# yabebalFantaye/MCEvidence

Measured on AMD Instinct MI355X. Metric: knn_queries_per_sec, higher is better.
Workload: dtype f16 filter + f64 refine (exact f64 results)

## Files before the change

### mcevidence_amd/csrc/capi_apo.hpp

```cpp
#pragma once
#include "sym_exchange.hpp"

namespace {

int pairs_once_plan(int64_t nr, int32_t d, int32_t kmax, Plan& p, bool quiet)
{
    if (kmax <= 1) return quiet ? MCE_ERR_INVALID : fail(MCE_ERR_INVALID, "kmax=%d must exceed k0=1", kmax);
    SameSetHint hint(true);
    const int rc = make_plan(nr, nr, d, kmax - 1, MCE_SELF_EXCLUDE, p);
    if (rc != MCE_OK) return rc;
    if (p.prune || !p.sym || p.twopass || !p.vh || !p.vh->launch_panel)
        return quiet ? MCE_ERR_INVALID : fail(MCE_ERR_INVALID, "pairs-once partition: this shape does not take the one-pass symmetric sweep");
    return MCE_OK;
}

struct PairsOnceShape {
    int nsplit = 1, panel = 0;
    size_t off_d = 0, off_i = 0;
    size_t total = 0;
};
PairsOnceShape pairs_once_shape(const Plan& p, int64_t nr, int32_t kmax, int32_t nparts)
{
    PairsOnceShape sh;
    const int nown = (p.nqblk + nparts - 1) / std::max(nparts, 1);
    const int env_split = env_pairs_once_split();
    const int env_panel = env_pairs_once_panel();
    int S = std::min(8, std::max(1, (1536 + nown - 1) / std::max(nown, 1)));
    if (env_split) S = env_split;
    const int def_panel = kSymPanelChunks[p.KST];
    int panel = S > 1 ? (int)std::max<int64_t>(8, std::min<int64_t>(def_panel, p.nchunk / (2 * S))) : 0;
    if (env_panel) panel = env_panel;
    sh.nsplit = S;
    sh.panel = panel;
    size_t off = p.total + dotp_ws_bytes(nr, kmax);
    if (S > 1) {
        off = align_up(off, 256);
        sh.off_d = off;
        off = align_up(off + (size_t)S * p.KCAP * (size_t)p.nq_pad * sizeof(double), 256);
        sh.off_i = off;
        off = align_up(off + (size_t)S * p.KCAP * (size_t)p.nq_pad * sizeof(int), 256);
    } else {
        sh.off_d = p.off_pd;
        sh.off_i = p.off_pi;
    }
    sh.total = off;
    return sh;
}
struct ApoCall { int64_t nr; int d, kmax, part, nparts, nsplit, panel, phase; };
std::mutex g_apo_mutex;
std::unordered_map<const void*, ApoCall> g_apo_calls;
int apo_step(const void* ws, int64_t nr, int d, int kmax, int part, int nparts, const PairsOnceShape& sh, int phase_from, int phase_to, int phase_set,
             const char* what)
{
    std::lock_guard<std::mutex> lk(g_apo_mutex);
    auto it = g_apo_calls.find(ws);
    if (phase_from > 0) {
        if (it == g_apo_calls.end())
            return fail(MCE_ERR_INVALID, "pairs-once partition: %s on a workspace that mce_pairs_once_prepare_dev has not prepared", what);
        const ApoCall& c = it->second;
        if (c.nr != nr || c.d != d || c.kmax != kmax || c.part != part || c.nparts != nparts || c.nsplit != sh.nsplit || c.panel != sh.panel)
            return fail(MCE_ERR_INVALID, "pairs-once partition: %s with other arguments than the workspace was prepared with (prepared: nr=%lld d=%d kmax=%d part %d "
                        "of %d, %d chains, panel %d)", what, (long long)c.nr, c.d, c.kmax, c.part, c.nparts, c.nsplit, c.panel);
        if (c.phase < phase_from || c.phase > phase_to)
            return fail(MCE_ERR_INVALID, "pairs-once partition: %s out of order (the calls are prepare, sweep, export, finish; this workspace stands after step %d)",
                        what, c.phase);
    }
    if (phase_set < 0) { if (it != g_apo_calls.end()) g_apo_calls.erase(it); }
    else g_apo_calls[ws] = ApoCall{nr, d, kmax, part, nparts, sh.nsplit, sh.panel, phase_set};
    return MCE_OK;
}
enum PairsOnceStep { kApoPrepare, kApoSweep, kApoExport, kApoFinish };
int pairs_once_begin(PairsOnceStep step, const void* ws, size_t ws_bytes, int64_t nr, int32_t d, int32_t kmax, int32_t part, int32_t nparts, Plan& p,
                     PairsOnceShape& sh)
{
    static const struct { int from, to, set; const char* what; } kSteps[4] = {{0, 0, 1, "prepare"}, {1, 1, 2, "sweep"}, {2, 3, 3, "export"},
                                                                               {2, 3, -1, "finish"}};
    int rc = pairs_once_plan(nr, d, kmax, p, false);
    if (rc != MCE_OK) return rc;
    if (nparts > p.nqblk || (step == kApoExport && nparts < 2))
        return step == kApoExport ? fail(MCE_ERR_INVALID, "part %d of %d", part, nparts)
                                  : fail(MCE_ERR_INVALID, "pairs-once partition: %d ranks for %d blocks", nparts, p.nqblk);
    sh = pairs_once_shape(p, nr, kmax, nparts);
    if (ws_bytes < sh.total)
        return step >= kApoExport ? fail(MCE_ERR_WORKSPACE, "workspace too small") : fail(MCE_ERR_WORKSPACE, "workspace too small: %zu < %zu", ws_bytes, sh.total);
    rc = apo_step(ws, nr, d, kmax, part, nparts, sh, kSteps[step].from, kSteps[step].to, kSteps[step].set, kSteps[step].what);
    if (rc != MCE_OK) return rc;
    p.apo = true; p.apo_nsplit = sh.nsplit; p.apo_panel = sh.panel; p.off_pd = sh.off_d; p.off_pi = sh.off_i;
    p.part = part; p.nparts = nparts;
    return MCE_OK;
}

__global__ __launch_bounds__(256) void pairs_once_fill_kernel(unsigned long long* __restrict__ p, int64_t n, unsigned long long v)
{
    for (int64_t i = (int64_t)blockIdx.x * 256 + threadIdx.x; i < n; i += (int64_t)gridDim.x * 256) p[i] = v;
}
__global__ __launch_bounds__(256) void pairs_once_row_gates_kernel(unsigned long long* __restrict__ thr, unsigned* __restrict__ rrow, float* __restrict__ rtile,
                                                                   const double* __restrict__ qinfo, const double* __restrict__ params, int64_t nq, int KST)
{
    const int64_t q = (int64_t)blockIdx.x * 256 + threadIdx.x;
    float R = 0.0f;
    if (q < nq) {
        R = mce::f16_row_gate_of(__longlong_as_double((long long)thr[q]), qinfo[2 * q], params, KST);
        rrow[q] = __float_as_uint(R);
    } else {
        thr[q] = 0x7FF0000000000000ull;
        rrow[q] = 0u;
    }
    float m = R;
#pragma unroll
    for (int o = 16; o >= 1; o >>= 1) m = fmaxf(m, __shfl_xor(m, o, 64));
    if ((threadIdx.x & 31) == 0) rtile[q >> 5] = m;
}

__global__ void pairs_once_poison_kernel(const int* __restrict__ err, double* __restrict__ dotp, int kmax)
{
    if (*err != 0 && (int)threadIdx.x < kmax) dotp[threadIdx.x] = __builtin_nan("");
}
__global__ __launch_bounds__(256) void pairs_once_check_kernel(const mce::SymEntry* __restrict__ recv, int64_t n, int qpb, int nqblk, int part, int nparts,
                                                               int* __restrict__ err)
{
    const int64_t i = (int64_t)blockIdx.x * 256 + threadIdx.x;
    if (i >= n) return;
    const int jb = recv[i].row / qpb;
    if (recv[i].row < 0 || jb >= nqblk || jb % nparts != part) *err = 1;
}

}

extern "C" {

int32_t mce_pairs_once_blocks(int64_t nr, int32_t d, int32_t kmax)
{
    Plan p;
    if (pairs_once_plan(nr, d, kmax, p, true) != MCE_OK) return 0;
    return p.nqblk;
}

size_t mce_pairs_once_workspace_bytes(int64_t nr, int32_t d, int32_t kmax, int32_t nparts)
{
    Plan p;
    if (nparts < 2 || pairs_once_plan(nr, d, kmax, p, true) != MCE_OK) return 0;
    return pairs_once_shape(p, nr, kmax, nparts).total;
}

int mce_pairs_once_prepare_dev(const double* dY, int64_t nr, int32_t d, int32_t kmax, int32_t part, int32_t nparts, size_t* bounds_offset,
                               int64_t* bounds_count, void* ws, size_t ws_bytes, void* stream)
{
    if (!dY || !ws || !bounds_offset || !bounds_count) return fail(MCE_ERR_INVALID, "null pointer argument");
    if (nparts < 2 || part < 0 || part >= nparts) return fail(MCE_ERR_INVALID, "part %d of %d (the pairs-once partition needs two ranks or more)", part, nparts);
    Plan p;
    PairsOnceShape sh;
    int rc = pairs_once_begin(kApoPrepare, ws, ws_bytes, nr, d, kmax, part, nparts, p, sh);
    if (rc != MCE_OK) return rc;
    hipStream_t st = static_cast<hipStream_t>(stream);
    char* wsc = static_cast<char*>(ws);
    p.apo_phase = 1;
    const unsigned long long inf_bits = 0x7FF0000000000000ull;
    hipLaunchKernelGGL(pairs_once_fill_kernel, dim3(1024), dim3(256), 0, st, reinterpret_cast<unsigned long long*>(wsc + p.off_sym + p.sl.thr), p.nq_pad, inf_bits);
    MCE_HIP(hipGetLastError());
    hipLaunchKernelGGL(pairs_once_fill_kernel, dim3(2048), dim3(256), 0, st, reinterpret_cast<unsigned long long*>(wsc + p.off_sym + p.sl.slots),
                       p.nq_pad * (int64_t)p.KCAP, inf_bits);
    MCE_HIP(hipGetLastError());
    if (sh.nsplit > 1) {
        static_assert(mce::f16_qpb(4) == 512, "one workgroup per block of list columns");
        hipLaunchKernelGGL(mce::sym_chain_init_kernel, dim3((unsigned)mce::apo_rank_count(p.nqblk, part, nparts)), dim3(512), 0, st,
                           reinterpret_cast<double*>(wsc + sh.off_d), reinterpret_cast<int*>(wsc + sh.off_i), p.nq_pad, p.KCAP, sh.nsplit, (int)part, (int)nparts);
        MCE_HIP(hipGetLastError());
    }
    SameSetHint hint(true);
    rc = run_search(p, dY, nr, dY, nr, d, kmax - 1, MCE_SELF_EXCLUDE, 0, wsc, st);
    if (rc != MCE_OK) return rc;
    *bounds_offset = p.off_sym + p.sl.thr;
    *bounds_count = p.nq_pad;
    return MCE_OK;
}

int mce_pairs_once_sweep_dev(const double* dY, int64_t nr, int32_t d, int32_t kmax, int32_t part, int32_t nparts, int64_t* d_counts,
                             int32_t* d_flags, void* ws, size_t ws_bytes, void* stream)
{
    if (!dY || !d_counts || !d_flags || !ws) return fail(MCE_ERR_INVALID, "null pointer argument");
    if (nparts < 2 || part < 0 || part >= nparts) return fail(MCE_ERR_INVALID, "part %d of %d (the pairs-once partition needs two ranks or more)", part, nparts);
    Plan p;
    PairsOnceShape sh;
    int rc = pairs_once_begin(kApoSweep, ws, ws_bytes, nr, d, kmax, part, nparts, p, sh);
    if (rc != MCE_OK) return rc;
    hipStream_t st = static_cast<hipStream_t>(stream);
    char* wsc = static_cast<char*>(ws);
    p.apo_phase = 2;
    const mce::KnnF16Args a = sym_args(p, wsc, nr, d, kmax - 1, 1);
    hipLaunchKernelGGL(pairs_once_row_gates_kernel, dim3((unsigned)(p.nq_pad / 256)), dim3(256), 0, st, a.sym.thr, a.sym.rrow, a.sym.rtile, a.qinfo, a.params, nr, p.KST);
    MCE_HIP(hipGetLastError());
    SameSetHint hint(true);
    rc = run_search(p, dY, nr, dY, nr, d, kmax - 1, MCE_SELF_EXCLUDE, 0, wsc, st);
    if (rc != MCE_OK) return rc;
    if (!p.sym_active) return fail(MCE_ERR_INVALID, "pairs-once partition: the sweep did not run");
    int* offs = reinterpret_cast<int*>(wsc + p.off_sym + p.sl.keys_a);
    static_assert(sizeof(long long) == sizeof(int64_t), "counts");
    hipLaunchKernelGGL(mce::apo_offsets_kernel, dim3(1), dim3(mce::kApoScanThreads), 0, st, a.sym.bucket_cnt, a.sym.bucket_flag, a.sym.cap, p.nqblk, (int)part,
                       (int)nparts, offs, reinterpret_cast<long long*>(d_counts), d_flags);
    MCE_HIP(hipGetLastError());
    return MCE_OK;
}

int mce_pairs_once_export_dev(int64_t nr, int32_t d, int32_t kmax, int32_t part, int32_t nparts, void* d_send, void* ws, size_t ws_bytes, void* stream)
{
    if (!ws) return fail(MCE_ERR_INVALID, "null pointer argument");
    Plan p;
    PairsOnceShape sh;
    const int rc = pairs_once_begin(kApoExport, ws, ws_bytes, nr, d, kmax, part, nparts, p, sh);
    if (rc != MCE_OK) return rc;
    if (!d_send) return MCE_OK;
    hipStream_t st = static_cast<hipStream_t>(stream);
    char* wsc = static_cast<char*>(ws);
    const mce::KnnF16Args a = sym_args(p, wsc, nr, d, kmax - 1, 1);
    const int* offs = reinterpret_cast<const int*>(wsc + p.off_sym + p.sl.keys_a);
    hipLaunchKernelGGL(mce::apo_export_kernel, dim3((unsigned)p.nqblk), dim3(256), 0, st, a.sym.bucket, offs, a.sym.cap, p.nqblk, (int)nparts,
                       static_cast<mce::SymEntry*>(d_send));
    MCE_HIP(hipGetLastError());
    return MCE_OK;
}

int mce_pairs_once_finish_dev(const double* dY, int64_t nr, int32_t d, int32_t kmax, int32_t part, int32_t nparts, const double* d_w,
                              const double* d_fs, const void* d_recv, int64_t nrecv, const int32_t* d_flags, double* d_dotp, void* ws,
                              size_t ws_bytes, void* stream)
{
    if (!dY || !d_w || !d_fs || !d_dotp || !d_flags || !ws || (nrecv > 0 && !d_recv)) return fail(MCE_ERR_INVALID, "null pointer argument");
    if (nparts < 2 || part < 0 || part >= nparts || nrecv < 0) return fail(MCE_ERR_INVALID, "part %d of %d, %lld entries", part, nparts, (long long)nrecv);
    Plan p;
    PairsOnceShape sh;
    int rc = pairs_once_begin(kApoFinish, ws, ws_bytes, nr, d, kmax, part, nparts, p, sh);
    if (rc != MCE_OK) return rc;
    hipStream_t st = static_cast<hipStream_t>(stream);
    char* wsc = static_cast<char*>(ws);
    const int K = kmax - 1;
    mce::KnnF16Args a = sym_args(p, wsc, nr, d, K, 1);
    const int nown = mce::apo_rank_count(p.nqblk, part, nparts);
    int* err = reinterpret_cast<int*>(wsc + p.off_sym + p.sl.keys_a) + p.nqblk + 1;
    MCE_HIP(mce::zero_async(err, sizeof(int), st));
    const int qpb = mce::f16_qpb(p.KCAP);
    if (nrecv > 0) {
        const unsigned nb = (unsigned)((nrecv + 255) / 256);
        hipLaunchKernelGGL(pairs_once_check_kernel, dim3(nb), dim3(256), 0, st, static_cast<const mce::SymEntry*>(d_recv), nrecv, qpb, p.nqblk, (int)part, (int)nparts, err);
        MCE_HIP(hipGetLastError());
        hipLaunchKernelGGL(mce::apo_import_kernel, dim3(nb), dim3(256), 0, st, static_cast<const mce::SymEntry*>(d_recv), nrecv, a.sym.bucket, a.sym.bucket_cnt,
                           a.sym.bucket_flag, a.sym.cap, qpb, p.nqblk, (int)part, (int)nparts);
        MCE_HIP(hipGetLastError());
    }
    hipLaunchKernelGGL(mce::apo_flags_kernel, dim3((unsigned)((nown + 255) / 256)), dim3(256), 0, st, d_flags, a.sym.bucket_flag, p.nqblk, (int)part, (int)nparts);
    MCE_HIP(hipGetLastError());
    a.seed_cfg = 0;
    MCE_HIP(p.vh->launch_sym_repair(a, st));
    if (sh.nsplit > 1 && nown > 0) {
        hipLaunchKernelGGL(mce::sym_chain_clear_kernel, dim3((unsigned)nown), dim3(512), 0, st, a.sym.bucket_flag, a.part_d, a.part_i, p.nq_pad, p.KCAP, sh.nsplit, (int)part, (int)nparts);
        MCE_HIP(hipGetLastError());
    }
    MCE_HIP(launch_sym_merge(p.KCAP, a.part_d, a.part_i, p.nq_pad, a.sym, part, p.nqblk, st, nparts));
    hipLaunchKernelGGL(mce::apo_iota_kernel, dim3((unsigned)((p.nqblk + 255) / 256)), dim3(256), 0, st, a.sym.done, p.nqblk);
    MCE_HIP(hipGetLastError());
    p.sym_qb_lo = 0; p.sym_qb_hi = p.nqblk; p.sym_active = true; p.L = sh.nsplit;
    double* partial = reinterpret_cast<double*>(wsc + p.total);
    rc = launch_merge(p, false, true, dY, dY, nr, d, K, MCE_SELF_EXCLUDE, 0, nullptr, nullptr, 1, (int)kmax, d_w, d_fs, partial, wsc, st);
    if (rc != MCE_OK) return rc;
    rc = finish_dotp(partial, (int64_t)nown * qpb, 1, kmax, d_dotp, st);
    if (rc != MCE_OK) return rc;
    hipLaunchKernelGGL(pairs_once_poison_kernel, dim3(1), dim3(64), 0, st, err, d_dotp, (int)kmax);
    MCE_HIP(hipGetLastError());
    return MCE_OK;
}

}
```

### mcevidence_amd/csrc/capi_common.hpp

```cpp
#pragma once
namespace {

thread_local char g_err[512] = "";
thread_local char g_last_kernel[256] = "";
thread_local int g_prof_on = 0;
thread_local std::vector<std::pair<hipEvent_t, hipEvent_t>> g_ev_pool;
thread_local size_t g_ev_used = 0;
thread_local size_t g_ev_calls = 0;
thread_local bool g_in_tail = false;
thread_local int g_split_depth = 0;
thread_local double g_last_prune_geom[3] = {0, 0, 0};
thread_local double g_last_flops_main = 0.0, g_last_flops_all = 0.0;
thread_local std::vector<std::pair<hipEvent_t, hipEvent_t>> g_evs_pool;
thread_local size_t g_evs_used = 0;

int fail(int code, const char* fmt, ...)
{
    va_list ap;
    va_start(ap, fmt);
    vsnprintf(g_err, sizeof(g_err), fmt, ap);
    va_end(ap);
    return code;
}

#define MCE_HIP(call)                                                                              \
    do {                                                                                           \
        hipError_t e_ = (call);                                                                    \
        if (e_ != hipSuccess)                                                                      \
            return fail(MCE_ERR_HIP, "%s failed: %s (%s:%d)", #call, hipGetErrorString(e_), __FILE__, __LINE__); \
    } while (0)

std::atomic<int> g_mode{0};
std::atomic<int> g_prune_mode{0};
struct Tuning {
    bool sym_kernel_f16 = false, tail_split = true, prune_prof = false, wide = true;
    int spin_limit = 1 << 21, sym_bucket = 0, sym_panel = 0, sym_seed_rows = 0, sym_seed_share = 2, sym_seed_mode = -1;
    int f16_seed_rows = -1, f16_seed_share = -1, f16_seed_tg = -1, rsplit = 0, panel_debug = 0, sym_chains = 0;
    size_t feed_wave_bytes = 0;
};
Tuning read_tuning()
{
    Tuning t;
    auto num = [](const char* name, int dflt) { const char* e = getenv(name); return e ? atoi(e) : dflt; };
    const char* e = getenv("MCE_SYM_KERNEL");
    t.sym_kernel_f16 = e && strcmp(e, "f16") == 0;
    t.spin_limit = num("MCE_SYM_SPIN_LIMIT", 1 << 21);
    t.sym_bucket = num("MCE_SYM_BUCKET", 0);
    t.sym_panel = num("MCE_SYM_PANEL", 0);
    t.sym_chains = num("MCE_SYM_CHAINS", 0);
    t.sym_seed_rows = num("MCE_SYM_SEED_ROWS", 0);
    t.sym_seed_share = num("MCE_SYM_SEED_SHARE", 2);
    t.sym_seed_mode = num("MCE_SYM_SEED_MODE", -1);
    t.f16_seed_rows = num("MCE_F16_SEED_ROWS", -1);
    t.f16_seed_share = num("MCE_F16_SEED_SHARE", -1);
    t.f16_seed_tg = num("MCE_F16_SEED_TG", -1);
    t.rsplit = num("MCE_RSPLIT", 0);
    t.tail_split = num("MCE_TAIL_SPLIT", 1) != 0;
    t.wide = num("MCE_WIDE", 1) != 0;
    t.panel_debug = num("MCE_PANEL_DEBUG", 0);
    t.prune_prof = getenv("MCE_PRUNE_PROF") != nullptr;
    if ((e = getenv("MCE_FEED_WAVE_BYTES"))) t.feed_wave_bytes = (size_t)std::strtoull(e, nullptr, 10);
    return t;
}
std::atomic<int> g_sym_mode{-1};
int sym_mode()
{
    int m = g_sym_mode.load();
    if (m < 0) {
        const char* e = getenv("MCE_SYM");
        m = e ? atoi(e) : 0;
        if (m < 0 || m > 2) m = 0;
        g_sym_mode.store(m);
    }
    return m;
}
const char* env_prune_heavy() { return getenv("MCE_PRUNE_HEAVY"); }
const char* env_prune_lists() { return getenv("MCE_PRUNE_LISTS"); }
const char* env_prune_times() { return getenv("MCE_PRUNE_TIMES"); }
bool env_long_on() { static const bool v = [] { const char* e = getenv("MCE_LONG"); return !(e && e[0] == '0'); }(); return v; }
bool env_deep_on() { static const bool v = [] { const char* e = getenv("MCE_DEEP"); return !(e && e[0] == '0'); }(); return v; }
int env_feed_eig() { static const int v = [] { const char* e = getenv("MCE_FEED_EIG"); return e && !strcmp(e, "hip") ? 2 : 1; }(); return v; }
bool env_feed_upload_async() { static const bool v = [] { const char* e = getenv("MCE_FEED_UPLOAD"); return e && !strcmp(e, "async"); }(); return v; }
int env_pairs_once_split() { static const int v = [] { const char* e = getenv("MCE_PAIRS_ONCE_SPLIT"); const int n = e ? atoi(e) : 0; return (n >= 1 && n <= 8) ? n : 0; }(); return v; }
int env_pairs_once_panel() { static const int v = [] { const char* e = getenv("MCE_PAIRS_ONCE_PANEL"); const int n = e ? atoi(e) : 0; return n >= 1 ? n : 0; }(); return v; }
struct CallOptions { int search = -1, prune = -1, sym = -1, same_set = -1, verify = -1, eig = 0; };
thread_local CallOptions t_opt;
thread_local std::vector<CallOptions> t_opt_stack;
int eff_search_mode() { return t_opt.search >= 0 ? t_opt.search : g_mode.load(); }
int eff_prune_mode() { return t_opt.prune >= 0 ? t_opt.prune : g_prune_mode.load(); }
int eff_sym_mode() { return t_opt.sym >= 0 ? t_opt.sym : sym_mode(); }
constexpr int kVerifyDefaultRows = 256;
constexpr int64_t kVerifyAlwaysFrom = 65536;
constexpr int kVerifySmallEvery = 8;
int default_verify_rows()
{
    static const int v = [] {
        const char* e = getenv("MCE_VERIFY");
        if (!e || !*e) return kVerifyDefaultRows;
        const long n = strtol(e, nullptr, 10);
        return (int)std::max<long>(0, std::min<long>(n, 1 << 20));
    }();
    return v;
}
bool verify_env_set() { static const bool s = [] { const char* e = getenv("MCE_VERIFY"); return e && *e; }(); return s; }
std::atomic<int> g_last_verify_rows{0};
thread_local unsigned t_small_search_count = 0;
int eff_verify(bool filter_path, int64_t nq)
{
    if (t_opt.verify >= 0) return t_opt.verify;
    if (!filter_path) return 0;
    if (nq < kVerifyAlwaysFrom && !verify_env_set() && (t_small_search_count++ % kVerifySmallEvery) != 0) return 0;
    return default_verify_rows();
}
constexpr int kSymAutoMinBlocks[5] = {0, 768, 257, 193, 193};
constexpr int kSymMaxChains = 8;
constexpr int kSymSeedMode[5] = {0, 0, 1, 1, 1};
constexpr int kSymPartitionMaxParts = 4;
thread_local int g_same_set_hint = -1;
thread_local size_t t_plan_cap = 0;
struct PlanCap {
    size_t prev;
    explicit PlanCap(size_t cap) : prev(t_plan_cap) { t_plan_cap = cap; }
    ~PlanCap() { t_plan_cap = prev; }
};
thread_local bool t_no_heavy = false;
struct NoHeavy {
    bool prev;
    NoHeavy() : prev(t_no_heavy) { t_no_heavy = true; }
    ~NoHeavy() { t_no_heavy = prev; }
};
struct SameSetHint {
    int prev;
    explicit SameSetHint(bool same) : prev(g_same_set_hint) { g_same_set_hint = same ? 1 : 0; }
    ~SameSetHint() { g_same_set_hint = prev; }
};
constexpr int kSymPanelChunks[5] = {0, 96, 256, 256, 256};
int sym_bucket_per_row(int K)
{
    const int b = read_tuning().sym_bucket;
    return b > 0 ? b : 6 * K + 24;
}
constexpr int64_t kPruneAutoMinQueries = 32768;
constexpr int64_t kPruneAutoMinRows[16] = {0, 100000, 100000, 100000, 100000, 125000, 150000, 250000, 500000, 0, 0, 0, 0, 0, 0, 0};

constexpr size_t kPoolMaxBytes = (size_t)64 << 20;
constexpr int kPoolSlots = 16;
struct PoolSlot { void* p = nullptr; size_t cap = 0; int dev = -1; bool busy = false; };
struct Pool {
    PoolSlot slot[kPoolSlots];
    PoolSlot& operator[](int i) { return slot[i]; }
    void release_idle()
    {
        for (int i = 0; i < kPoolSlots; ++i)
            if (slot[i].p && !slot[i].busy) {
                int cur = 0;
                (void)hipGetDevice(&cur);
                if (slot[i].dev != cur) (void)hipSetDevice(slot[i].dev);
                (void)hipFree(slot[i].p);
                if (slot[i].dev != cur) (void)hipSetDevice(cur);
                slot[i] = PoolSlot();
            }
    }
    ~Pool() { release_idle(); }
};
thread_local Pool g_pool;

struct PinnedArena {
    void* p = nullptr;
    size_t cap = 0;
    void release()
    {
        if (p) (void)hipHostFree(p);
        p = nullptr;
        cap = 0;
    }
    hipError_t reserve(size_t n)
    {
        if (n <= cap) return hipSuccess;
        release();
        const size_t c = std::max<size_t>(n + n / 2, (size_t)64 << 10);
        hipError_t e = hipHostMalloc(&p, c, hipHostMallocPortable);
        if (e != hipSuccess) { p = nullptr; return e; }
        cap = c;
        return hipSuccess;
    }
    ~PinnedArena() { release(); }
};
thread_local PinnedArena g_pinned;

thread_local const double* g_last_params = nullptr;

struct DevBuf {
    void* p = nullptr;
    int slot = -1;
    ~DevBuf()
    {
        if (p && g_last_params >= static_cast<const double*>(p) &&
            reinterpret_cast<const char*>(g_last_params) < static_cast<const char*>(p) + bytes)
            g_last_params = nullptr;
        if (slot >= 0) g_pool[slot].busy = false;
        else if (p) (void)hipFree(p);
    }
    size_t bytes = 0;
    hipError_t alloc(size_t n)
    {
        if (n == 0) n = 1;
        bytes = n;
        if (n <= kPoolMaxBytes) {
            int dev = 0;
            (void)hipGetDevice(&dev);
            int pick = -1;
            for (int i = 0; i < kPoolSlots; ++i)
                if (!g_pool[i].busy && g_pool[i].p && g_pool[i].dev == dev && g_pool[i].cap >= n &&
                    (pick < 0 || g_pool[i].cap < g_pool[pick].cap)) pick = i;
            if (pick < 0)
                for (int i = 0; i < kPoolSlots; ++i)
                    if (!g_pool[i].busy) {
                        if (g_pool[i].p) { (void)hipFree(g_pool[i].p); g_pool[i].p = nullptr; g_pool[i].cap = 0; }
                        const size_t cap = n + n / 4;
                        hipError_t e = hipMalloc(&g_pool[i].p, cap);
                        if (e != hipSuccess) { g_pool[i].p = nullptr; return e; }
                        g_pool[i].cap = cap;
                        g_pool[i].dev = dev;
                        pick = i;
                        break;
                    }
            if (pick >= 0) {
                g_pool[pick].busy = true;
                slot = pick;
                p = g_pool[pick].p;
                return hipSuccess;
            }
        }
        return hipMalloc(&p, n);
    }
    template <class T> T* as() { return static_cast<T*>(p); }
};

}
```

### mcevidence_amd/csrc/capi_plan.hpp

```cpp
#pragma once
namespace {

using mce::kMaxDevices;
constexpr int kAssumedCUs = 256;

size_t align_up(size_t x, size_t a) { return (x + a - 1) / a * a; }

constexpr bool kPruneHeavyDefault = false;
constexpr int kPruneHeavyMinBlocks = 64, kPruneHeavyCount = 700, kPruneHeavyMaxShare = 16, kPruneHeavyMinCount = 32, kPruneHeavyMaxRounds = 60;
constexpr double kPruneHeavyFullRounds = 10.0;
constexpr int kPruneHeavySplit = 4, kPruneHeavyMaxSplit = 8;
constexpr int kPruneWaveQueries = mce::kHQT * 32;
constexpr int kWideMinBlocks = 480;
bool prune_heavy_enabled()
{
    if (t_no_heavy) return false;
    const char* e = env_prune_heavy();
    return kPruneHeavyDefault || (e && *e && strcmp(e, "0") != 0);
}
static_assert(mce::kPruneWavesPerBlock == mce::kHWaves, "prune.hip orders kHWaves waves per query block");

constexpr int kRefineMargin = 2;
struct Plan {
    const mce::KnnVariant* v = nullptr;
    const mce::KnnF16Variant* vh = nullptr;
    const mce::KnnDeepVariant* vd = nullptr;
    bool filter() const { return vh != nullptr || vd != nullptr; }
    const mce::KnnLongVariant* vl = nullptr;
    size_t off_xf = 0, off_xn = 0;
    bool generic = false;
    int KST = 0;
    size_t off_yh = 0, off_xh = 0, off_qinfo = 0, off_params = 0;
    int KS = 0, KCAP = 0, QT = 0, CT = 0;
    int64_t nchunk = 0;
    int64_t nrow_pad = 0;
    int nqblk = 0;
    int64_t nq_pad = 0;
    int rsplit = 1;
    int L = 4;
    size_t off_yf = 0, off_pd = 0, off_pi = 0, off_center = 0, off_msum = 0, total = 0;
    double cost = 0.0;
    int ksel = 0;
    bool twopass = false;
    bool wide_ok = false;
    bool prune = false;
    bool kd_ready = false;
    int part = 0, nparts = 1;
    int sym_qb_lo = 0, sym_qb_hi = 0;
    bool apo = false;
    int apo_phase = 0;
    int apo_nsplit = 1;
    int apo_panel = 0;
    int64_t pl_nr = 0;
    mce::PruneLayout pl;
    size_t off_prune = 0;
    size_t off_heavy = 0;
    int heavy_max = 0;
    bool sym = false;
    bool sym_active = false;
    mce::SymLayout sl;
    size_t off_sym = 0;
    int sym_nsplit = 1;
    int sym_panel = 0;
};

const mce::KnnVariant* variant_for(int KS, int kcap_idx)
{
    switch (kcap_idx) {
        case 0: return &mce::g_knn_kcap4[mce::mfma_variant_index(KS)];
        case 1: return &mce::g_knn_kcap8[mce::mfma_variant_index(KS)];
        case 2: return &mce::g_knn_kcap12[mce::mfma_variant_index(KS)];
        case 3: return &mce::g_knn_kcap16[mce::mfma_variant_index(KS)];
        case 4: return &mce::g_knn_kcap24[mce::mfma_variant_index(KS)];
        default: return &mce::g_knn_kcap32[mce::mfma_variant_index(KS)];
    }
}

int sweep_seed_cfg(int64_t cps, int CT, int kneed)
{
    const Tuning t = read_tuning();
    if (t.f16_seed_rows >= 0 || t.f16_seed_share >= 0 || t.f16_seed_tg >= 0)
        return mce::f16_seed_cfg(cps, CT, kneed, t.f16_seed_rows >= 0 ? t.f16_seed_rows : MCE_H_SEED_ROWS, t.f16_seed_share >= 0 ? t.f16_seed_share : MCE_H_SEED_SHARE,
                                 t.f16_seed_tg >= 0 ? t.f16_seed_tg : MCE_H_SEED_TG);
    for (int share = MCE_H_SEED_SHARE; share >= 2; share /= 2)
        for (int tg = MCE_H_SEED_TG; tg >= 2; tg /= 2)
            if (const int cfg = mce::f16_seed_cfg(cps, CT, kneed, MCE_H_SEED_ROWS, share, tg)) return cfg;
    return 0;
}

template <class V> const V* by_kcap(int ki, const V* t4, const V* t8, const V* t12, const V* t16) { return ki == 0 ? t4 : ki == 1 ? t8 : ki == 2 ? t12 : t16; }

double split_cost(const Plan& p, bool filt, int64_t nr, int32_t K, int r)
{
    const double n_r = (double)nr / r;
    const double lnf = 1.0 + std::log(std::max(1.0, n_r / K));
    const double block = filt ? 64.0 * p.QT * p.KST * (n_r / 32.0) + 300.0 * 32.0 * p.QT * K * lnf
                              : 256.0 * p.KS * (n_r / 16.0) + 1000.0 * 32.0 * K * lnf;
    const double rounds = std::ceil((double)p.nqblk * r / kAssumedCUs);
    return rounds * block;
}

int make_plan(int64_t nq, int64_t nr, int32_t d, int32_t K, int32_t self_mode, Plan& p)
{
    if (nq < 0 || nr < 1 || d < 1 || K < 1) return fail(MCE_ERR_INVALID, "invalid sizes nq=%lld nr=%lld d=%d K=%d", (long long)nq, (long long)nr, d, K);
    if (self_mode < 0 || self_mode > 2) return fail(MCE_ERR_INVALID, "invalid self_mode %d", self_mode);
    if (d > mce::kGenMaxDim) return fail(MCE_ERR_DIM_RANGE, "d=%d exceeds the supported maximum %d", d, mce::kGenMaxDim);
    if (K > mce::kGenMaxK) return fail(MCE_ERR_K_RANGE, "K=%d exceeds the supported maximum %d", K, mce::kGenMaxK);
    const int64_t usable = (self_mode == MCE_SELF_EXCLUDE) ? nr - 1 : nr;
    if (K > usable)
        return fail(MCE_ERR_K_RANGE, "Expected n_neighbors <= n_samples_fit, but n_neighbors = %d, n_samples_fit = %lld", K, (long long)usable);
    if (nr >= (int64_t)1 << 31) return fail(MCE_ERR_INVALID, "nr=%lld exceeds 2^31-1 reference rows", (long long)nr);

    const bool wide_f64 = d > MCE_MAX_DIM && d <= mce::kWideMaxDim && K <= MCE_MAX_K;
    if (env_long_on() && d >= mce::kLongMinDim && d <= mce::kLongMaxDim && K <= MCE_MAX_K) {
        p.ksel = std::min<int>(K + kRefineMargin, MCE_MAX_K);
        p.vl = &mce::g_knn_long[p.ksel <= 8 ? 0 : (p.ksel <= 16 ? 1 : 2)];
        p.v = nullptr;
        p.vh = nullptr;
        p.KCAP = p.vl->kcap;
        p.CT = p.vl->ct;
        p.QT = mce::kLongQT;
        p.KS = mce::long_ksp(d);
        p.nqblk = (int)std::max<int64_t>(1, (nq + mce::kLongQPB - 1) / mce::kLongQPB);
        p.nq_pad = (int64_t)p.nqblk * mce::kLongQPB;
        const int64_t rows_per_chunk = (int64_t)p.CT * 16;
        p.nchunk = (nr + rows_per_chunk - 1) / rows_per_chunk;
        p.nrow_pad = p.nchunk * rows_per_chunk;
        int best_r = 1;
        double best_c = 1e300;
        const int rmax = (int)std::min<int64_t>(mce::kMaxLists, p.nchunk);
        for (int r = 1; r <= rmax; ++r) {
            const double c = std::ceil((double)p.nqblk * r / kAssumedCUs) * (std::ceil((double)p.nchunk / r) + 16.0);
            if (c < best_c * 0.98) { best_c = c; best_r = r; }
        }
        p.rsplit = best_r;
        p.L = p.rsplit;
        p.cost = best_c;
        p.pl_nr = nr;
        size_t off = 0;
        p.off_pd = off;
        off = align_up(off + (size_t)p.L * p.KCAP * (size_t)p.nq_pad * sizeof(double), 256);
        p.off_pi = off;
        off = align_up(off + (size_t)p.L * p.KCAP * (size_t)p.nq_pad * sizeof(int), 256);
        p.off_center = off;
        off = align_up(off + (size_t)(d + 4) * sizeof(double), 256);
        p.off_msum = off;
        off = align_up(off + (size_t)mce::kLongMeanBlocks * (size_t)d * sizeof(double), 256);
        p.off_yf = off;
        off = align_up(off + (size_t)p.nrow_pad * (size_t)p.KS * 4 * sizeof(double), 256);
        p.off_xf = off;
        off = align_up(off + (size_t)p.nq_pad * (size_t)p.KS * 4 * sizeof(double), 256);
        p.off_xn = off;
        off = align_up(off + (size_t)p.nq_pad * sizeof(double), 256);
        p.total = off + 256;
        return MCE_OK;
    }
    if ((d > MCE_MAX_DIM && !wide_f64) || K > MCE_MAX_K) {
        p.generic = true;
        p.v = nullptr;
        p.vh = nullptr;
        p.KCAP = K;
        p.rsplit = 1;
        p.L = 1;
        p.nqblk = (int)std::max<int64_t>(1, (nq + mce::kGenThreads - 1) / mce::kGenThreads);
        p.nq_pad = (int64_t)p.nqblk * mce::kGenThreads;
        size_t off = 0;
        p.off_pd = off;
        off = align_up(off + (size_t)K * (size_t)p.nq_pad * sizeof(double), 256);
        p.off_pi = off;
        off = align_up(off + (size_t)K * (size_t)p.nq_pad * sizeof(int), 256);
        p.off_center = off;
        off = align_up(off + (size_t)nq * K * sizeof(double), 256);
        p.off_msum = off;
        p.total = off + 256;
        return MCE_OK;
    }
    p.KS = mce::mfma_ks_for(d);
    int ki = 0;
    while (ki < mce::kNumKcap - 1 && mce::kKcapList[ki] < K) ++ki;
    p.KCAP = mce::kKcapList[ki];
    const bool f16 = !wide_f64 && (eff_search_mode() != 1) && mce::f16_supported(d, K);
    const bool deep = wide_f64 && (eff_search_mode() != 1) && mce::deep_supported(d, K) && env_deep_on();
    const bool filt = f16 || deep;
    p.vd = nullptr;
    int qpb, rows_per_tile;
    if (filt) {
        if (K > 16) {
            p.twopass = true;
            ki = 3;
            p.KCAP = 16;
        }
        if (deep) {
            p.KST = mce::deep_ksteps(d);
            p.vd = &by_kcap(ki, mce::g_knn_deep_kcap4, mce::g_knn_deep_kcap8, mce::g_knn_deep_kcap12, mce::g_knn_deep_kcap16)[p.KST == 5 ? 0 : (p.KST == 6 ? 1 : 2)];
            p.vh = nullptr;
            p.QT = mce::kHQT;
            p.CT = p.vd->ct;
        } else {
            p.KST = mce::f16_ksteps(d);
            p.vh = &by_kcap(ki, mce::g_knn_f16_kcap4, mce::g_knn_f16_kcap8, mce::g_knn_f16_kcap12, mce::g_knn_f16_kcap16)[p.KST - 1];
            p.QT = p.vh->qt;
            p.CT = p.vh->ct;
        }
        p.v = nullptr;
        qpb = mce::f16_qpb(p.KCAP);
        rows_per_tile = 32;
    } else {
        p.ksel = std::min<int>(K + kRefineMargin, MCE_MAX_K);
        p.pl_nr = nr;
        ki = 0;
        while (ki < mce::kNumKcap - 1 && mce::kKcapList[ki] < p.ksel) ++ki;
        p.KCAP = mce::kKcapList[ki];
        p.v = variant_for(p.KS, ki);
        p.vh = nullptr;
        p.QT = p.v->qt;
        p.CT = p.v->ct;
        qpb = mce::queries_per_block(p.QT);
        rows_per_tile = 16;
    }
    p.nqblk = (int)std::max<int64_t>(1, (nq + qpb - 1) / qpb);
    p.wide_ok = f16 && !p.twopass && p.KST == 1 && p.vh->launch_wide && p.nqblk >= kWideMinBlocks && nr <= ((int64_t)1 << 25) && read_tuning().wide;
    if (p.wide_ok && (p.nqblk & 1)) p.nqblk += 1;
    p.nq_pad = (int64_t)p.nqblk * qpb;
    const int64_t rows_per_chunk = (int64_t)p.CT * rows_per_tile;
    p.nchunk = (nr + rows_per_chunk - 1) / rows_per_chunk;
    p.nrow_pad = p.nchunk * rows_per_chunk;

    if (f16 && !p.twopass && p.KST == 1 && d <= mce::kPruneMaxDim && p.vh->launch_prune && nq > 0 &&
        p.nrow_pad <= ((int64_t)1 << mce::kHRelBits) && (int64_t)p.nqblk * p.nchunk <= mce::kPruneMaxPairs) {
        const int pm = eff_prune_mode();
        p.prune = pm == 2 || (pm == 0 && kPruneAutoMinRows[d] > 0 && nr >= kPruneAutoMinRows[d] && nq >= kPruneAutoMinQueries &&
                                           nq >= nr / 8);
    }
    if (p.prune) {
        p.CT = mce::kHPruneChunkTiles;
        p.nchunk = (nr + p.CT * 32 - 1) / (p.CT * 32);
        p.nrow_pad = p.nchunk * p.CT * 32;
        if (p.nrow_pad > ((int64_t)1 << mce::kHRelBits)) p.prune = false;
        if (!p.prune) {
            p.CT = p.vh->ct;
            p.nchunk = (nr + rows_per_chunk - 1) / rows_per_chunk;
            p.nrow_pad = p.nchunk * rows_per_chunk;
        }
    }
    int best_r = 1;
    double best_c = 1e300;
    const int rmax = (int)std::min<int64_t>(p.twopass ? mce::kMaxLists / 2 : mce::kMaxLists, p.nchunk);
    const int rmin = f16 ? (int)((nr + ((int64_t)1 << mce::kHRelBits) - 1) >> mce::kHRelBits) : 1;
    if (deep && p.nrow_pad > ((int64_t)1 << mce::kHRelBits))
        return fail(MCE_ERR_INVALID, "reference set too large for the fp16-filter path at d = %d (nr=%lld): use search mode 1", d, (long long)nr);
    if (rmin > rmax) return fail(MCE_ERR_INVALID, "reference set too large for the fp16-filter path (nr=%lld)", (long long)nr);
    for (int r = std::max(1, rmin); r <= rmax; ++r) {
        const double c = split_cost(p, filt, nr, K, r);
        if (c < best_c * 0.98) { best_c = c; best_r = r; }
    }
    if (f16 && !p.twopass && p.nqblk <= kAssumedCUs) {
        const int kneed = K + 1;
        for (int r = std::min(rmax, kAssumedCUs / p.nqblk); r >= std::max(1, rmin); --r)
            if (sweep_seed_cfg(p.nchunk / r, p.CT, kneed)) { best_r = r; break; }
    }
    if (deep && p.nqblk <= kAssumedCUs) {
        for (int r = std::min(rmax, kAssumedCUs / p.nqblk); r >= 1; --r)
            if ((p.nchunk / r) * p.CT >= 4 * (K + 1)) { best_r = r; break; }
    }
    if (const int r = read_tuning().rsplit) {
        if (r >= std::max(1, rmin) && r <= rmax) best_r = r;
    }
    if (p.prune) best_r = 1;
    p.rsplit = best_r;
    p.cost = split_cost(p, filt, nr, K, best_r);
    auto layout = [&]() {
    p.L = p.twopass ? 2 * p.rsplit : p.rsplit;

    size_t off = 0;
    p.off_yf = off;
    if (filt) {
        p.off_yh = off;
        off = align_up(off + (size_t)p.nrow_pad * (size_t)(16 * p.KST) * 2, 256);
        p.off_xh = off;
        off = align_up(off + (size_t)p.nq_pad * (size_t)(16 * p.KST) * 2, 256);
        p.off_qinfo = off;
        off = align_up(off + (size_t)p.nq_pad * 2 * sizeof(double), 256);
        p.off_params = off;
        off = align_up(off + (size_t)mce::HP_COUNT * sizeof(double), 256);
    } else {
        off = align_up(off + (size_t)p.nrow_pad * (size_t)(4 * p.KS) * sizeof(double), 256);
    }
    if (f16 && (!p.twopass || p.vh->launch_panel_lower) && !p.prune && nq == nr && p.vh->launch_sym && p.nqblk >= 2 && p.nrow_pad <= ((int64_t)1 << mce::kHSymRowBits)) {
        const int sm = eff_sym_mode();
        p.sym = sm == 2 || (sm == 0 && p.nqblk >= kSymAutoMinBlocks[p.KST] * ((p.KST == 1 && p.KCAP == 16) ? 2 : 1));
        if (g_same_set_hint == 0 || (g_same_set_hint < 0 && t_opt.same_set == 0)) p.sym = false;
    }
    p.sym_nsplit = 1;
    p.sym_panel = 0;
    if (p.sym && !p.twopass) {
        const Tuning tun = read_tuning();
        int S = 1;
        if (tun.sym_chains >= 1) S = std::min(tun.sym_chains, kSymMaxChains);
        p.sym_nsplit = S;
        if (S > 1) p.sym_panel = (int)std::max<int64_t>(8, std::min<int64_t>(kSymPanelChunks[p.KST], p.nchunk / (2 * S)));
    }
    const int l_alloc = std::max(p.L, p.sym_nsplit);
    p.off_pd = off;
    off = align_up(off + (size_t)l_alloc * p.KCAP * (size_t)p.nq_pad * sizeof(double), 256);
    p.off_pi = off;
    off = align_up(off + (size_t)l_alloc * p.KCAP * (size_t)p.nq_pad * sizeof(int), 256);
    p.off_center = off;
    off = align_up(off + (size_t)3 * mce::kMaxDimPad * sizeof(double), 256);
    p.off_msum = off;
    off = align_up(off + (size_t)mce::kMeanBlocks * mce::kStatStride * sizeof(double), 256);
    if (p.prune) {
        mce::prune_layout(nq, p.nq_pad, p.nqblk, nr, p.nrow_pad, p.nchunk, d, p.pl);
        p.pl_nr = nr;
        p.off_prune = off;
        off = align_up(off + p.pl.total, 256);
        if (nq == nr && p.nqblk >= kPruneHeavyMinBlocks && prune_heavy_enabled()) {
            p.heavy_max = std::max(p.nqblk * mce::kHWaves / kPruneHeavyMaxShare, kPruneHeavyMinCount);
            p.off_heavy = off;
            off = align_up(off + (size_t)p.heavy_max * kPruneWaveQueries * (kPruneHeavyMaxSplit - 1) * p.KCAP * (sizeof(double) + sizeof(int)), 256);
        }
    }
    if (p.sym) {
        mce::sym_layout(nr, p.nq_pad, p.nqblk, d, p.KCAP, mce::f16_qpb(p.KCAP), sym_bucket_per_row(std::min<int>(K, p.KCAP)), p.sl);
        p.off_sym = off;
        off = align_up(off + p.sl.total, 256);
    }
    p.total = off;
    };
    layout();
    while (t_plan_cap && p.total > t_plan_cap && p.rsplit > std::max(1, rmin)) {
        p.rsplit -= 1;
        layout();
    }
    return MCE_OK;
}

size_t dotp_ws_bytes(int64_t nq, int32_t kmax)
{
    const int64_t nb = (nq + mce::kRedThreads - 1) / mce::kRedThreads;
    return align_up((size_t)std::max<int64_t>(nb, 1) * (size_t)kmax * sizeof(double), 256);
}

int plan_for_workspace(int64_t nq, int64_t nr, int32_t d, int32_t K, int32_t self_mode, size_t ws_bytes, size_t extra, bool same_set_fallback,
                       Plan& p, std::optional<NoHeavy>& nh)
{
    int rc = make_plan(nq, nr, d, K, self_mode, p);
    if (rc != MCE_OK) return rc;
    if (same_set_fallback && ws_bytes < p.total + extra && p.sym) {
        g_same_set_hint = 0;
        rc = make_plan(nq, nr, d, K, self_mode, p);
        if (rc != MCE_OK) return rc;
    }
    if (ws_bytes < p.total + extra && p.heavy_max > 0) {
        nh.emplace();
        rc = make_plan(nq, nr, d, K, self_mode, p);
        if (rc != MCE_OK) return rc;
    }
    if (ws_bytes < p.total + extra) return fail(MCE_ERR_WORKSPACE, "workspace too small: %zu < %zu", ws_bytes, p.total + extra);
    return MCE_OK;
}

}
```

### mcevidence_amd/csrc/capi_search.hpp

```cpp
#pragma once
namespace {

double ln_unit_ball(int d) { return 0.5 * d * std::log(M_PI) - std::lgamma(1.0 + 0.5 * d); }

hipError_t launch_sym_merge(int KCAP, double* pd, int* pi, int64_t nq_pad, const mce::SymParams& sym, int qb_lo, int qb_hi, hipStream_t st, int stride = 1)
{
    const int nb = qb_hi > qb_lo ? (qb_hi - qb_lo + stride - 1) / stride : 0;
    if (nb <= 0) return hipSuccess;
    const dim3 g((unsigned)nb), b(mce::kSymMergeThreads);
    static_assert(mce::kSymMergeThreads == mce::f16_qpb(4), "one merge block per query block");
    switch (KCAP) {
        case 4: hipLaunchKernelGGL(mce::sym_merge_kernel<4>, g, b, 0, st, pd, pi, nq_pad, sym.bucket_cnt, sym.bucket_flag, sym.bucket, sym.cap, qb_lo, stride); break;
        case 8: hipLaunchKernelGGL(mce::sym_merge_kernel<8>, g, b, 0, st, pd, pi, nq_pad, sym.bucket_cnt, sym.bucket_flag, sym.bucket, sym.cap, qb_lo, stride); break;
        case 12: hipLaunchKernelGGL(mce::sym_merge_kernel<12>, g, b, 0, st, pd, pi, nq_pad, sym.bucket_cnt, sym.bucket_flag, sym.bucket, sym.cap, qb_lo, stride); break;
        default: hipLaunchKernelGGL(mce::sym_merge_kernel<16>, g, b, 0, st, pd, pi, nq_pad, sym.bucket_cnt, sym.bucket_flag, sym.bucket, sym.cap, qb_lo, stride); break;
    }
    return hipGetLastError();
}

struct KernelBracket {
    bool on = false; hipStream_t st = nullptr;
    hipError_t begin() const
    {
        if (!on) return hipSuccess;
        if (g_ev_used == g_ev_pool.size()) {
            hipEvent_t e0, e1;
            if (const hipError_t e = hipEventCreate(&e0)) return e;
            if (const hipError_t e = hipEventCreate(&e1)) return e;
            g_ev_pool.emplace_back(e0, e1);
        }
        return hipEventRecord(g_ev_pool[g_ev_used].first, st);
    }
    hipError_t end() const
    {
        if (!on) return hipSuccess;
        if (const hipError_t e = hipEventRecord(g_ev_pool[g_ev_used].second, st)) return e;
        ++g_ev_used;
        if (!g_in_tail) ++g_ev_calls;
        return hipSuccess;
    }
};
struct SearchBracket {
    hipStream_t st; bool on;
    SearchBracket(hipStream_t s, bool o) : st(s), on(o)
    {
        if (!on) return;
        if (g_evs_used == g_evs_pool.size()) {
            hipEvent_t e0, e1;
            if (hipEventCreate(&e0) != hipSuccess || hipEventCreate(&e1) != hipSuccess) { on = false; return; }
            g_evs_pool.emplace_back(e0, e1);
        }
        (void)hipEventRecord(g_evs_pool[g_evs_used].first, st);
    }
    ~SearchBracket() { if (on) { (void)hipEventRecord(g_evs_pool[g_evs_used].second, st); ++g_evs_used; } }
};

size_t list_set(const Plan& p, int set) { return (size_t)set * p.KCAP * (size_t)p.nq_pad; }

mce::KnnF16Args f16_args(const Plan& p, char* ws, const double* X, int64_t nq, const double* Y, int64_t nr, int32_t d, int32_t K, int self_exclude,
                         int64_t self_offset)
{
    mce::KnnF16Args a;
    a.Yh = ws + p.off_yh; a.nchunk_total = p.nchunk; a.rsplit = p.rsplit; a.Xh = ws + p.off_xh;
    a.qinfo = reinterpret_cast<const double*>(ws + p.off_qinfo); a.params = reinterpret_cast<const double*>(ws + p.off_params);
    a.X = X; a.Y = Y; a.nq = nq; a.nr = nr; a.D = d; a.nq_pad = p.nq_pad; a.nqblk = p.nqblk;
    a.self_exclude = self_exclude; a.self_offset = self_offset; a.ksel = K;
    a.part_d = reinterpret_cast<double*>(ws + p.off_pd); a.part_i = reinterpret_cast<int*>(ws + p.off_pi);
    return a;
}
mce::KnnF16Args sym_args(const Plan& p, char* ws, int64_t n, int32_t d, int32_t K, int self_exclude)
{
    char* const sw = ws + p.off_sym;
    const double* rows = reinterpret_cast<const double*>(sw + p.sl.Ys);
    mce::KnnF16Args a = f16_args(p, ws, rows, n, rows, n, d, K, self_exclude, 0);
    a.rsplit = 1;
    a.rperm = reinterpret_cast<const int*>(sw + p.sl.perm);
    a.sym.thr = reinterpret_cast<unsigned long long*>(sw + p.sl.thr);
    a.sym.rrow = reinterpret_cast<unsigned*>(sw + p.sl.rrow);
    a.sym.rtile = reinterpret_cast<float*>(sw + p.sl.rtile);
    a.sym.slots = reinterpret_cast<unsigned long long*>(sw + p.sl.slots);
    a.sym.bucket_cnt = reinterpret_cast<int*>(sw + p.sl.bucket_cnt);
    a.sym.bucket_flag = reinterpret_cast<int*>(sw + p.sl.bucket_flag);
    a.sym.bucket = reinterpret_cast<mce::SymEntry*>(sw + p.sl.bucket);
    a.sym.cap = p.sl.cap;
    a.sym.done = reinterpret_cast<int*>(sw + p.sl.done);
    const Tuning tun = read_tuning();
    a.sym.panel = tun.sym_panel > 0 ? tun.sym_panel : kSymPanelChunks[p.KST];
    return a;
}

struct F16Search {
    const double* sX = nullptr;
    const double* sY = nullptr;
    mce::PruneOut po;
    bool use_sym = false;
};

struct Search {
    Plan& p;
    const double* dX; int64_t nq; const double* dY; int64_t nr; int32_t d, K;
    int32_t self_mode; int64_t self_offset; char* ws; hipStream_t st;
    int phase;
    double* pd; int* pi;
    double* center; double* msum;
    int self_exclude;
    KernelBracket kb;
    int generic(), long_rows(), deep(), fp64();
    int f16_prepare(F16Search& f), pruned(const F16Search& f), symmetric(), f16_sweep(const F16Search& f);
};

int Search::generic()
{
    const size_t lds = mce::generic_lds_bytes();
    hipLaunchKernelGGL(mce::knn_generic_kernel, dim3((unsigned)p.nqblk), dim3(mce::kGenThreads), 0, st, dX, nq, dY, nr, (int)d,
                       (int)K, p.nq_pad, self_exclude, self_offset, pd, pi);
    MCE_HIP(hipGetLastError());
    snprintf(g_last_kernel, sizeof(g_last_kernel), "knn_generic_kernel grid=%d block=%d lds=%zu", p.nqblk, mce::kGenThreads, lds);
    return MCE_OK;
}

int Search::long_rows()
{
    const int threads = 256;
    double* yf = reinterpret_cast<double*>(ws + p.off_yf);
    double* xf = reinterpret_cast<double*>(ws + p.off_xf);
    double* xn = reinterpret_cast<double*>(ws + p.off_xn);
    hipLaunchKernelGGL(mce::pack_refs_kernel, dim3((unsigned)((p.nrow_pad + threads - 1) / threads)), dim3(threads), 0, st, dY, nr, (int)d, p.KS, p.nrow_pad, center, yf);
    MCE_HIP(hipGetLastError());
    const int64_t qe = p.nq_pad * (int64_t)p.KS;
    hipLaunchKernelGGL(mce::long_pack_queries_kernel, dim3((unsigned)((qe + 255) / 256)), dim3(256), 0, st, dX, nq, (int)d, p.KS, p.nq_pad, center, xf);
    MCE_HIP(hipGetLastError());
    hipLaunchKernelGGL(mce::long_query_norms_kernel, dim3((unsigned)((p.nq_pad + 255) / 256)), dim3(256), 0, st, dX, nq, (int)d, p.nq_pad, center, xn);
    MCE_HIP(hipGetLastError());
    mce::LongArgs a;
    a.Yf = yf; a.Xf = xf; a.xn = xn;
    a.nchunk_total = p.nchunk; a.rsplit = p.rsplit; a.KSP = p.KS; a.KSB = mce::long_ksb(d);
    a.nq = nq; a.nq_pad = p.nq_pad; a.nqblk = p.nqblk;
    a.self_exclude = self_exclude; a.self_offset = self_offset; a.ksel = p.ksel > K ? p.ksel : K;
    a.part_d = pd; a.part_i = pi;
    MCE_HIP(kb.begin());
    MCE_HIP(p.vl->launch(a, st));
    MCE_HIP(kb.end());
    snprintf(g_last_kernel, sizeof(g_last_kernel), "%s grid=%d block=%d lds=%zu qt=%d ct=%d rsplit=%d ksp=%d", p.vl->name, p.nqblk * p.rsplit, mce::kThreads,
             p.vl->lds_bytes, p.QT, p.CT, p.rsplit, p.KS);
    g_last_flops_main = g_last_flops_all = (double)p.nq_pad * (double)p.nrow_pad * 2.0 * 4.0 * p.KS;
    return MCE_OK;
}

int Search::deep()
{
    _Float16* yh = reinterpret_cast<_Float16*>(ws + p.off_yh);
    _Float16* xh = reinterpret_cast<_Float16*>(ws + p.off_xh);
    double* qinfo = reinterpret_cast<double*>(ws + p.off_qinfo);
    double* params = reinterpret_cast<double*>(ws + p.off_params);
    MCE_HIP(mce::zero_async(params, mce::HP_COUNT * sizeof(double), st));
    const bool separate_queries = !(dX >= dY && dX + (size_t)nq * d <= dY + (size_t)nr * d);
    hipLaunchKernelGGL(mce::f16_radius_rows_kernel, dim3((unsigned)std::min<int64_t>((nr + 255) / 256, 2048)), dim3(256), 0, st, dY, nr, (int)d, center, params);
    MCE_HIP(hipGetLastError());
    if (separate_queries && nq > 0) {
        hipLaunchKernelGGL(mce::f16_radius_rows_kernel, dim3((unsigned)std::min<int64_t>((nq + 255) / 256, 2048)), dim3(256), 0, st, dX, nq, (int)d, center, params);
        MCE_HIP(hipGetLastError());
    }
    hipLaunchKernelGGL(mce::f16_scale_from_radius_kernel, dim3(1), dim3(1), 0, st, params);
    MCE_HIP(hipGetLastError());
    const int64_t rows_per_block = 4 * (64 / (2 * p.KST));
    const int64_t pack_blocks = std::min<int64_t>((p.nrow_pad + rows_per_block - 1) / rows_per_block, 2048);
    hipLaunchKernelGGL(mce::f16_pack_refs_kernel, dim3((unsigned)pack_blocks), dim3(256), 0, st, dY, nr, (int)d, p.KST, p.nrow_pad, center, params, yh);
    MCE_HIP(hipGetLastError());
    hipLaunchKernelGGL(mce::f16_pack_queries_kernel, dim3((unsigned)((p.nq_pad + rows_per_block - 1) / rows_per_block)), dim3(256), 0, st,
                       dX, nq, p.nq_pad, (int)d, p.KST, center, params, xh, qinfo);
    MCE_HIP(hipGetLastError());
    mce::DeepArgs a;
    a.Yh = yh; a.Xh = xh; a.qinfo = qinfo; a.params = params; a.X = dX; a.Y = dY; a.part_d = pd; a.part_i = pi;
    a.nq = nq; a.nr = nr; a.nq_pad = p.nq_pad; a.self_offset = self_offset; a.nchunk_total = p.nchunk;
    a.D = d; a.ksel = K; a.self_exclude = self_exclude; a.nqblk = p.nqblk; a.rsplit = p.rsplit;
    const Tuning tun = read_tuning();
    a.debug = tun.panel_debug;
    const int64_t tiles_split = (p.nchunk / p.rsplit) * p.CT;
    const int64_t want = (tun.f16_seed_rows >= 0 ? tun.f16_seed_rows : MCE_H_SEED_ROWS) / 32;
    auto tg_for = [&](int G) {
        int64_t tg = std::min<int64_t>(want, tiles_split / 4) / G;
        if (tg < 1) tg = std::min<int64_t>(want, tiles_split / 2) / G;
        return (int)std::max<int64_t>(tg, 0);
    };
    a.seed_tg = tg_for(K + a.self_exclude);
    MCE_HIP(kb.begin());
    double seed_rows = (double)a.seed_tg * (K + a.self_exclude) * 32.0 * p.rsplit;
    if (p.twopass) {
        const int tg2 = a.seed_tg;
        a.ksel = 16;
        a.seed_groups = 16 + a.self_exclude;
        a.seed_tg = tg_for(a.seed_groups);
        const int tg1 = a.seed_tg;
        MCE_HIP(p.vd->launch(a, st));
        a.lo_d = pd; a.lo_i = pi;
        a.part_d = pd + list_set(p, p.rsplit); a.part_i = pi + list_set(p, p.rsplit);
        a.ksel = K - 16;
        a.seed_groups = K + a.self_exclude;
        a.seed_tg = tg2;
        MCE_HIP(p.vd->launch_lower(a, st));
        seed_rows = ((double)tg1 * (16 + a.self_exclude) + (double)tg2 * (K + a.self_exclude)) * 32.0 * p.rsplit;
    } else {
        MCE_HIP(p.vd->launch(a, st));
    }
    MCE_HIP(kb.end());
    g_last_flops_main = g_last_flops_all = (double)p.nq_pad * ((p.twopass ? 2.0 : 1.0) * (double)p.nrow_pad + seed_rows) * 2.0 * 16.0 * p.KST;
    snprintf(g_last_kernel, sizeof(g_last_kernel), "%s grid=%d block=%d lds=%zu qt=%d ct=%d rsplit=%d%s seed=%dx%d", p.vd->name, p.nqblk * p.rsplit, mce::kHThreads,
             p.vd->lds_bytes, p.QT, p.CT, p.rsplit, p.twopass ? " two passes" : "", K + a.self_exclude, a.seed_tg);
    return MCE_OK;
}

int Search::f16_prepare(F16Search& f)
{
    _Float16* yh = reinterpret_cast<_Float16*>(ws + p.off_yh);
    _Float16* xh = reinterpret_cast<_Float16*>(ws + p.off_xh);
    double* qinfo = reinterpret_cast<double*>(ws + p.off_qinfo);
    double* params = reinterpret_cast<double*>(ws + p.off_params);
    double* box_y = center + mce::kMaxDimPad;
    double* box_x = center + 2 * mce::kMaxDimPad;
    if (phase != 2) MCE_HIP(mce::zero_async(params, mce::HP_COUNT * sizeof(double), st));
    bool separate_queries = !(dX >= dY && dX + (size_t)nq * d <= dY + (size_t)nr * d);
    f.sX = dX; f.sY = dY;
    f.use_sym = p.sym && dX == dY && nq == nr && self_offset == 0 && g_split_depth == 0;
    if (f.use_sym) {
        if (phase != 2) MCE_HIP(mce::sym_prepare(dY, nr, (int)d, center, p.nq_pad, ws + p.off_sym, p.sl, st));
        f.sX = f.sY = reinterpret_cast<const double*>(ws + p.off_sym + p.sl.Ys);
        separate_queries = false;
    }
    if (p.prune) {
        const bool same_set = (dX == dY && nq == nr);
        MCE_HIP(mce::prune_prepare(dX, nq, dY, nr, (int)d, same_set, mce::f16_qpb(p.KCAP), p.CT * 32, p.nq_pad, p.nqblk, p.nrow_pad,
                                   p.nchunk, ws + p.off_prune, p.pl, st, f.po, p.kd_ready && same_set));
        f.sX = f.po.Xs; f.sY = f.po.Ys;
        separate_queries = separate_queries && !same_set;
    }
    if (separate_queries) {
        hipLaunchKernelGGL(mce::col_stats_partial_kernel, dim3(mce::kMeanBlocks), dim3(mce::kMeanThreads), 0, st, dX, nq, (int)d, msum);
        MCE_HIP(hipGetLastError());
        hipLaunchKernelGGL(mce::f16_box_about_kernel, dim3(1), dim3(64), 0, st, msum, (int)d, center, box_x);
        MCE_HIP(hipGetLastError());
    }
    if (phase == 2) return MCE_OK;
    hipLaunchKernelGGL(mce::f16_scale_kernel, dim3(1), dim3(64), 0, st, box_y, separate_queries ? box_x : (const double*)nullptr, params);
    MCE_HIP(hipGetLastError());
    const int64_t rows_per_block = 4 * (64 / (2 * p.KST));
    const int64_t pack_blocks = std::min<int64_t>((p.nrow_pad + rows_per_block - 1) / rows_per_block, 2048);
    const bool one_pass = f.sX == f.sY && nq == nr && p.nq_pad <= p.nrow_pad;
    hipLaunchKernelGGL(mce::f16_pack_refs_kernel, dim3((unsigned)pack_blocks), dim3(256), 0, st,
                       f.sY, nr, (int)d, p.KST, p.nrow_pad, center, params, yh, one_pass ? xh : (_Float16*)nullptr, one_pass ? qinfo : (double*)nullptr,
                       one_pass ? p.nq_pad : (int64_t)0);
    MCE_HIP(hipGetLastError());
    if (!one_pass) {
        hipLaunchKernelGGL(mce::f16_pack_queries_kernel, dim3((unsigned)((p.nq_pad + rows_per_block - 1) / rows_per_block)), dim3(256), 0, st,
                           f.sX, nq, p.nq_pad, (int)d, p.KST, center, params, xh, qinfo);
        MCE_HIP(hipGetLastError());
    }
    return MCE_OK;
}

int Search::pruned(const F16Search& f)
{
    const mce::PruneOut& po = f.po;
    mce::KnnF16Args a = f16_args(p, ws, f.sX, nq, f.sY, nr, d, K, self_exclude, self_offset);
    a.clist = po.clist; a.cdist = po.cdist; a.list_len = (int)p.nchunk; a.rperm = po.rperm; a.qperm = po.qperm;
    a.tbox_r = po.tbox_r; a.tbox_q = po.tbox_q; a.cbox_r = po.cbox_r; a.border = po.border;
    const int nw_total = p.nqblk * mce::kHWaves;
    if (p.nparts > 1) { a.qblk0 = p.part; a.qblk_stride = p.nparts; a.nqblk_run = (nw_total - p.part + p.nparts - 1) / p.nparts; }
    const int nblk_run = a.nqblk_run ? a.nqblk_run : nw_total;
    int hv_n = 0, hv_S = 1;
    if (p.heavy_max > 0 && dX == dY && nq == nr) {
        const double rounds = (double)nblk_run / 2048.0;
        const char* hv_env = env_prune_heavy();
        if ((kPruneHeavyDefault || (hv_env && !strcmp(hv_env, "auto"))) && rounds < kPruneHeavyMaxRounds) {
            const double fr = std::min(1.0, kPruneHeavyFullRounds / std::max(rounds, 1.0));
            hv_n = std::min(std::max((int)(kPruneHeavyCount * fr), kPruneHeavyMinCount), std::min(p.heavy_max, nblk_run));
            hv_S = kPruneHeavySplit;
        }
        if (const char* e = hv_env) {
            int n_ = hv_n, s_ = kPruneHeavySplit;
            if (sscanf(e, "%d,%d", &n_, &s_) >= 1) { hv_n = std::min(std::max(n_, 0), std::min(p.heavy_max, nblk_run)); hv_S = std::min(std::max(s_, 1), kPruneHeavyMaxSplit); }
        }
        if (hv_n == 0 || hv_S == 1) { hv_n = 0; hv_S = 1; }
    }
    double* hv_d = reinterpret_cast<double*>(ws + p.off_heavy);
    int* hv_i = reinterpret_cast<int*>(hv_d + (size_t)p.heavy_max * kPruneWaveQueries * (kPruneHeavyMaxSplit - 1) * p.KCAP);
    a.seed_cfg = hv_n | (hv_S << 24);
    a.lo_d = hv_n ? hv_d : nullptr; a.lo_i = hv_n ? hv_i : nullptr;
    const char* times_file = env_prune_times();
    const size_t n_wg = (size_t)(nblk_run + hv_n * (hv_S - 1));
    DevBuf wg_times;
    if (times_file && *times_file) { MCE_HIP(wg_times.alloc(n_wg * sizeof(float))); a.wg_us = wg_times.as<float>(); }
    MCE_HIP(kb.begin());
    const char* force_lists = env_prune_lists();
    mce::knn_f16_launch_fn short_fn = nullptr;
    int short_lc = 0;
    if (p.vh->launch_prune_short && K <= p.vh->prune_short_lc) { short_fn = p.vh->launch_prune_short; short_lc = p.vh->prune_short_lc; }
    else if (p.vh->launch_prune_short2 && K <= p.vh->prune_short_lc2) { short_fn = p.vh->launch_prune_short2; short_lc = p.vh->prune_short_lc2; }
    const bool short_lists = short_fn && !(force_lists && !strcmp(force_lists, "long"));
    MCE_HIP(short_lists ? short_fn(a, st) : p.vh->launch_prune(a, st));
    MCE_HIP(kb.end());
    if (a.wg_us) {
        std::vector<float> us(n_wg);
        MCE_HIP(hipStreamSynchronize(st));
        MCE_HIP(hipMemcpy(us.data(), a.wg_us, n_wg * sizeof(float), hipMemcpyDeviceToHost));
        if (FILE* fh = fopen(times_file, "wb")) {
            const int hdr[4] = {(int)n_wg, hv_n, hv_S, 1};
            fwrite(hdr, sizeof(int), 4, fh);
            fwrite(us.data(), sizeof(float), n_wg, fh);
            fclose(fh);
        }
    }
    if (hv_n) {
        const unsigned fb = (unsigned)(((int64_t)hv_n * kPruneWaveQueries + mce::kRedThreads - 1) / mce::kRedThreads);
        hipLaunchKernelGGL(mce::prune_heavy_fold_kernel, dim3(fb), dim3(mce::kRedThreads), 0, st, pd, pi, p.nq_pad, p.KCAP, hv_d, hv_i, hv_n, hv_S,
                           kPruneWaveQueries, po.border, a.qblk0, a.qblk_stride);
        MCE_HIP(hipGetLastError());
    }
    g_last_params = a.params;
    g_last_flops_main = g_last_flops_all = -1.0;
    g_last_prune_geom[0] = p.nqblk; g_last_prune_geom[1] = (double)p.nchunk; g_last_prune_geom[2] = p.CT;
    snprintf(g_last_kernel, sizeof(g_last_kernel), "%s pruned grid=%d block=64 lds=%zu qt=%d ct=%d chunks=%lld heavy=%dx%d lists=%d", p.vh->name,
             nblk_run + hv_n * (hv_S - 1), mce::f16_prune_lds_bytes(p.KST, d, short_lists ? short_lc : p.KCAP), p.QT, p.CT, (long long)p.nchunk, hv_n,
             hv_S, short_lists ? short_lc : p.KCAP);
    return MCE_OK;
}

int sym_units_and_flops(const Plan& p, const mce::PanelGeom& g, bool panel_kernel, int64_t nr, int panel)
{
    int units = mce::sym_unit_count(p.nqblk, mce::kHWaves * mce::kHQT, panel * p.CT, (int)((nr + 31) / 32) + (int)(((nr + 31) / 32) & 1));
    double tiles = 0.0;
    if (panel_kernel) {
        units = mce::panel_unit_count(g);
        for (int u = 0; g_prof_on && u < units; ++u) {
            int pp, aa, lo, hi;
            mce::panel_unit_decode(u, g, pp, aa);
            mce::panel_unit_tiles(pp, aa, g, lo, hi);
            tiles += hi - lo;
        }
    } else {
        const double tpb = mce::kHWaves * mce::kHQT, T = (double)((nr + 31) / 32);
        for (int b = 0; b < p.nqblk; ++b) tiles += std::min(tpb * (b + 1), T);
    }
    g_last_flops_main = tiles * 16.0 * 1024.0 * 32.0 * p.KST;
    return units;
}

int Search::symmetric()
{
    char* const sw = ws + p.off_sym;
    mce::KnnF16Args a = sym_args(p, ws, nr, d, K, self_exclude);
    const Tuning tun = read_tuning();
    const int seed_rows = tun.sym_seed_rows > 0 ? tun.sym_seed_rows : (p.KST == 1 ? 65536 : 32768) * (p.apo && p.nparts >= 4 ? 2 : 1);
    const int seed_share = tun.sym_seed_share;
    auto sym_seed_for = [&](int kk) {
        int cfg = mce::f16_seed_cfg(p.nchunk, p.CT, kk + a.self_exclude, seed_rows, seed_share, MCE_H_SEED_TG);
        for (int tg = MCE_H_SEED_TG / 2; cfg == 0 && tg >= 1; tg /= 2)
            cfg = mce::f16_seed_cfg(p.nchunk, p.CT, kk + a.self_exclude, seed_rows, seed_share, tg);
        if (cfg) cfg |= ((tun.sym_seed_mode >= 0 ? tun.sym_seed_mode : kSymSeedMode[p.KST]) & 3) << 28;
        return cfg;
    };
    const int qb_lo = p.nparts > 1 && !p.apo ? (int)((int64_t)p.nqblk * p.part / p.nparts) : 0;
    const int qb_hi = p.nparts > 1 && !p.apo ? (int)((int64_t)p.nqblk * (p.part + 1) / p.nparts) : p.nqblk;
    p.sym_qb_lo = qb_lo; p.sym_qb_hi = qb_hi;
    const bool panel_kernel = !tun.sym_kernel_f16 || p.nparts > 1 || p.twopass;
    mce::PanelGeom geom;
    geom.qb_lo = qb_lo; geom.qb_hi = qb_hi; geom.tpb = mce::kHWaves * mce::kHQT; geom.ct = p.CT; geom.tpp = a.sym.panel * p.CT; geom.sym_on = 1;
    geom.ntiles = (int)((nr + 31) / 32) + (int)(((nr + 31) / 32) & 1);
    const bool apo = p.apo && p.nparts > 1 && !p.twopass && panel_kernel;
    const bool chains1 = !apo && p.nparts == 1 && panel_kernel && !p.twopass && p.sym_nsplit > 1;
    if (apo) { geom.blk_first = p.part; geom.blk_stride = p.nparts; }
    if (apo || chains1) {
        const int pn = apo ? p.apo_panel : p.sym_panel;
        if (pn > 0 && (apo || tun.sym_panel <= 0)) { a.sym.panel = pn; geom.tpp = a.sym.panel * p.CT; }
        geom.nsplit = std::max(1, apo ? p.apo_nsplit : p.sym_nsplit);
        if (geom.nsplit > 1) {
            a.sym.done = reinterpret_cast<int*>(sw + p.sl.keys_b);
            MCE_HIP(mce::zero_async(a.sym.done, (size_t)p.nqblk * geom.nsplit * sizeof(int), st));
            if (!apo) {
                hipLaunchKernelGGL(mce::sym_chain_init_kernel, dim3((unsigned)p.nqblk), dim3(512), 0, st, pd, pi, p.nq_pad, p.KCAP, geom.nsplit, 0, 1);
                MCE_HIP(hipGetLastError());
            }
        }
    }
    const bool unit_table = apo || geom.nsplit > 1;
    const int npass = p.twopass ? 2 : 1;
    int seed_used = 0;
    for (int pass = 0; pass < npass; ++pass) {
        const bool lower = pass == 1;
        const int Kp = !p.twopass ? K : (lower ? K - 16 : 16);
        double* const pdp = pd + (lower ? list_set(p, 1) : 0);
        int* const pip = pi + (lower ? list_set(p, 1) : 0);
        if (lower) {
            MCE_HIP(mce::zero_async(a.sym.bucket_cnt, (size_t)3 * p.nqblk * sizeof(int), st));
            a.sym.slot_stride = p.KCAP;
        }
        a.ksel = lower ? K : Kp;
        a.seed_cfg = sym_seed_for(a.ksel);
        a.part_d = pdp; a.part_i = pip;
        a.qblk0 = qb_lo;
        a.nqblk_run = qb_hi - qb_lo;
        if (apo) {
            a.qblk0 = p.part; a.qblk_stride = p.nparts; a.nqblk_run = mce::apo_rank_count(p.nqblk, p.part, p.nparts);
        }
        if (a.nqblk_run > 0 && phase != 2) MCE_HIP((lower ? p.vh->launch_sym_pre32 : p.vh->launch_sym_pre)(a, st));
        a.qblk0 = 0; a.qblk_stride = 1; a.nqblk_run = 0;
        if (phase == 1) return MCE_OK;
        if (pass == 0) seed_used = a.seed_cfg;
        a.seed_cfg = 0;
        a.ksel = Kp;
        a.lo_d = lower ? pd : nullptr; a.lo_i = lower ? pi : nullptr;
        if (pass == 0) MCE_HIP(kb.begin());
        if (panel_kernel) {
            mce::PanelArgs pa;
            pa.Yh = static_cast<const _Float16*>(a.Yh); pa.Xh = static_cast<const _Float16*>(a.Xh); pa.qinfo = a.qinfo; pa.params = a.params;
            pa.X = a.X; pa.Y = a.Y; pa.rperm = a.rperm;
            pa.part_d = pdp; pa.part_i = pip; pa.nq = nq; pa.nr = nr; pa.nq_pad = p.nq_pad; pa.self_offset = 0;
            pa.D = d; pa.ksel = Kp; pa.self_exclude = a.self_exclude; pa.spin_limit = tun.spin_limit;
            pa.sym = a.sym; pa.debug = tun.panel_debug; pa.geom = geom; pa.lo_d = a.lo_d; pa.lo_i = a.lo_i;
            if (unit_table) {
                const int nun = mce::panel_unit_count(geom);
                if ((size_t)nun * sizeof(mce::PanelUnit) > (size_t)p.nq_pad * sizeof(int)) return fail(MCE_ERR_INVALID, "symmetric sweep: %d units do not fit the table", nun);
                mce::PanelUnit* tab = reinterpret_cast<mce::PanelUnit*>(sw + p.sl.vals_a);
                if (nun > 0) {
                    hipLaunchKernelGGL(mce::panel_unit_table_kernel, dim3((unsigned)((nun + 255) / 256)), dim3(256), 0, st, geom, nun, tab);
                    MCE_HIP(hipGetLastError());
                }
                pa.units = tab;
            }
            MCE_HIP((lower ? p.vh->launch_panel_lower : p.vh->launch_panel)(pa, st));
        } else {
            MCE_HIP(p.vh->launch_sym(a, st));
        }
        if (pass == 0) MCE_HIP(kb.end());
        if (apo) break;
        MCE_HIP((lower ? p.vh->launch_sym_repair_lower : p.vh->launch_sym_repair)(a, st));
        if (geom.nsplit > 1) {
            hipLaunchKernelGGL(mce::sym_chain_clear_kernel, dim3((unsigned)p.nqblk), dim3(512), 0, st, a.sym.bucket_flag, pdp, pip, p.nq_pad, p.KCAP, geom.nsplit, 0, 1);
            MCE_HIP(hipGetLastError());
        }
        MCE_HIP(launch_sym_merge(p.KCAP, pdp, pip, p.nq_pad, a.sym, qb_lo, qb_hi, st));
    }
    p.sym_active = true;
    p.L = geom.nsplit > 1 ? geom.nsplit : npass;
    const int sym_units = sym_units_and_flops(p, geom, panel_kernel, nr, a.sym.panel);
    g_last_flops_all = g_last_flops_main + (double)(seed_used & 0xffff) * p.CT * (double)(qb_hi - qb_lo) * 16.0 * 1024.0 * 32.0 * p.KST;
    snprintf(g_last_kernel, sizeof(g_last_kernel), "%s symmetric%s%s%s grid=%d block=%d lds=%zu qt=%d ct=%d panel=%d seed=%dx%d/%d bucket=%d", p.vh->name, panel_kernel ? " panel-kernel" : "",
             p.twopass ? " two passes" : "", geom.blk_stride > 1 ? " pairs-once" : (geom.nsplit > 1 ? " chains" : ""), sym_units,
             mce::kHThreads, panel_kernel ? p.vh->lds_bytes_panel : p.vh->lds_bytes_sym, p.QT, p.CT, a.sym.panel, seed_used & 0xffff, (seed_used >> 16) & 0xfff, (seed_used >> 28) & 3, p.sl.cap);
    return MCE_OK;
}

int Search::f16_sweep(const F16Search& f)
{
    mce::KnnF16Args a = f16_args(p, ws, f.sX, nq, f.sY, nr, d, K, self_exclude, self_offset);
    auto seed_cfg = [&](int ksel) { return sweep_seed_cfg(p.nchunk / p.rsplit, p.CT, ksel + a.self_exclude); };
    MCE_HIP(kb.begin());
    if (p.twopass) {
        a.ksel = 16;
        a.seed_cfg = seed_cfg(16);
        MCE_HIP(p.vh->launch(a, st));
        a.lo_d = pd; a.lo_i = pi;
        a.part_d = pd + list_set(p, p.rsplit); a.part_i = pi + list_set(p, p.rsplit);
        a.ksel = K - 16;
        a.seed_cfg = 0;
        MCE_HIP(p.vh->launch_lower(a, st));
    } else {
        a.seed_cfg = seed_cfg(K);
        if (p.wide_ok) MCE_HIP(p.vh->launch_wide(a, st));
        else MCE_HIP(p.vh->launch(a, st));
    }
    MCE_HIP(kb.end());
    const int seed_first = p.twopass ? seed_cfg(16) : a.seed_cfg;
    g_last_flops_main = (double)p.nqblk * ((double)p.nchunk + (double)(seed_first & 0xffff) * p.rsplit) * p.CT * 16.0 * 1024.0 * 32.0 * p.KST +
                        (p.twopass ? (double)p.nqblk * (double)p.nchunk * p.CT * 16.0 * 1024.0 * 32.0 * p.KST : 0.0);
    g_last_flops_all = g_last_flops_main;
    char seed_txt[48] = "";
    if (seed_first) snprintf(seed_txt, sizeof(seed_txt), " seed=%dx%d", seed_first & 0xffff, seed_first >> 16);
    const bool wide = p.wide_ok && !p.twopass;
    snprintf(g_last_kernel, sizeof(g_last_kernel), "%s grid=%d block=%d lds=%zu qt=%d ct=%d rsplit=%d%s%s%s", p.vh->name,
             (wide ? p.nqblk / 2 : p.nqblk) * p.rsplit, mce::kHThreads, wide ? p.vh->lds_bytes_wide : p.vh->lds_bytes, wide ? 2 * p.QT : p.QT, p.CT, p.rsplit,
             p.twopass ? " two passes" : "", seed_txt, wide ? " wide" : "");
    return MCE_OK;
}

int Search::fp64()
{
    const int threads = 256;
    double* yf = reinterpret_cast<double*>(ws + p.off_yf);
    hipLaunchKernelGGL(mce::pack_refs_kernel, dim3((unsigned)((p.nrow_pad + threads - 1) / threads)), dim3(threads), 0, st, dY, nr,
                       (int)d, p.KS, p.nrow_pad, center, yf);
    MCE_HIP(hipGetLastError());
    mce::KnnArgs a;
    a.Yf = yf; a.nchunk_total = p.nchunk; a.rsplit = p.rsplit; a.X = dX; a.center = center; a.nq = nq; a.D = d;
    a.nq_pad = p.nq_pad; a.nqblk = p.nqblk; a.self_exclude = self_exclude; a.self_offset = self_offset;
    a.ksel = p.ksel > K ? p.ksel : K;
    a.part_d = pd; a.part_i = pi;
    MCE_HIP(kb.begin());
    MCE_HIP(p.v->launch(a, st));
    MCE_HIP(kb.end());
    snprintf(g_last_kernel, sizeof(g_last_kernel), "%s grid=%d block=%d lds=%zu qt=%d ct=%d rsplit=%d", p.v->name,
             p.nqblk * p.rsplit, mce::kThreads, p.v->lds_bytes, p.QT, p.CT, p.rsplit);
    g_last_flops_main = g_last_flops_all = (double)p.nq_pad * (double)p.nrow_pad * 2.0 * 4.0 * p.KS;
    return MCE_OK;
}

int run_search(Plan& p, const double* dX, int64_t nq, const double* dY, int64_t nr, int32_t d, int32_t K,
               int32_t self_mode, int64_t self_offset, char* ws, hipStream_t st)
{
    p.sym_active = false;
    const int phase = p.apo ? p.apo_phase : 0;
    double* center = reinterpret_cast<double*>(ws + p.off_center);
    double* msum = reinterpret_cast<double*>(ws + p.off_msum);
    Search s{p, dX, nq, dY, nr, d, K, self_mode, self_offset, ws, st, phase, reinterpret_cast<double*>(ws + p.off_pd), reinterpret_cast<int*>(ws + p.off_pi),
             center, msum, (self_mode == MCE_SELF_EXCLUDE) ? 1 : 0, KernelBracket{}};
    if (p.generic) return s.generic();
    if (p.vl) {
        hipLaunchKernelGGL(mce::long_col_mean_partial_kernel, dim3(mce::kLongMeanBlocks), dim3(256), 0, st, dY, nr, (int)d, mce::kLongMeanBlocks, msum);
        MCE_HIP(hipGetLastError());
        hipLaunchKernelGGL(mce::long_col_mean_final_kernel, dim3((unsigned)((d + 255) / 256)), dim3(256), 0, st, msum, nr, (int)d, mce::kLongMeanBlocks, center);
        MCE_HIP(hipGetLastError());
    } else if (d > MCE_MAX_DIM) {
        static_assert(3 * mce::kMaxDimPad >= 128 && mce::kStatStride >= 128, "wide column means");
        hipLaunchKernelGGL(mce::col_mean_wide_partial_kernel, dim3(mce::kMeanBlocks), dim3(256), 0, st, dY, nr, (int)d, msum);
        MCE_HIP(hipGetLastError());
        hipLaunchKernelGGL(mce::col_mean_wide_final_kernel, dim3(1), dim3(128), 0, st, msum, nr, (int)d, center);
        MCE_HIP(hipGetLastError());
    } else if (phase != 2) {
        hipLaunchKernelGGL(mce::col_stats_partial_kernel, dim3(mce::kMeanBlocks), dim3(mce::kMeanThreads), 0, st, dY, nr, (int)d, msum);
        MCE_HIP(hipGetLastError());
        hipLaunchKernelGGL(mce::col_stats_final_kernel, dim3(1), dim3(64), 0, st, msum, nr, (int)d, center, center + mce::kMaxDimPad);
        MCE_HIP(hipGetLastError());
    }
    const bool prof = g_prof_on && g_ev_used < 1024;
    SearchBracket search_bracket(st, prof && g_evs_used < 1024);
    g_last_flops_main = g_last_flops_all = 0.0;
    s.kb = KernelBracket{prof, st};
    if (p.vl) return s.long_rows();
    if (p.vd) return s.deep();
    if (!p.vh) return s.fp64();
    F16Search f;
    const int rc = s.f16_prepare(f);
    if (rc != MCE_OK) return rc;
    if (p.prune) return s.pruned(f);
    return f.use_sym ? s.symmetric() : s.f16_sweep(f);
}

int launch_merge(const Plan& p, bool write_dist, bool fuse, const double* dX, const double* dY, int64_t nq, int32_t d, int K,
                 int self_mode, int64_t self_offset, double* d_dist, int64_t* d_idx, int k0, int kmax,
                 const double* d_w, const double* d_fs, double* partial, char* ws, hipStream_t st)
{
    const bool same_set = (dX == dY && nq == p.pl_nr);
    const bool wave_parts = p.prune && p.nparts > 1 && !p.sym_active;
    const int qpb = wave_parts ? kPruneWaveQueries : (p.filter() ? mce::f16_qpb(p.KCAP) : 1);
    const int nunits = wave_parts ? p.nqblk * mce::kHWaves : p.nqblk;
    int64_t ncol = nq;
    int64_t col0 = 0, col1 = INT64_MAX;
    const int* border = p.prune ? reinterpret_cast<const int*>(ws + p.off_prune + p.pl.border) : nullptr;
    if (p.sym_active && p.nparts > 1 && p.apo) {
        ncol = (int64_t)((nunits - p.part + p.nparts - 1) / p.nparts) * qpb;
        border = reinterpret_cast<const int*>(ws + p.off_sym + p.sl.done);
    } else if (p.sym_active && p.nparts > 1) {
        col0 = (int64_t)p.sym_qb_lo * qpb;
        col1 = std::min<int64_t>((int64_t)p.sym_qb_hi * qpb, nq);
        ncol = std::max<int64_t>(col1 - col0, 0);
    } else if (p.nparts > 1) ncol = (int64_t)((nunits - p.part + p.nparts - 1) / p.nparts) * qpb;
    const unsigned blocks = (unsigned)std::max<int64_t>((ncol + mce::kRedThreads - 1) / mce::kRedThreads, 1);
    const double* pd = reinterpret_cast<const double*>(ws + p.off_pd);
    const int* pi = reinterpret_cast<const int*>(ws + p.off_pi);
    const bool refine = !p.filter() && !p.generic;
    const double lnc = fuse ? ln_unit_ball(d) : 0.0;
    const int* qperm = nullptr;
    if (p.prune) qperm = reinterpret_cast<const int*>(ws + p.off_prune + (same_set ? p.pl.perm_r : p.pl.perm_q));
    if (p.sym_active) qperm = reinterpret_cast<const int*>(ws + p.off_sym + p.sl.perm);
#define MCE_MERGE(W, F, R)                                                                                          \
    hipLaunchKernelGGL((mce::merge_lists_kernel<W, F, R>), dim3(blocks), dim3(mce::kRedThreads), 0, st, pd, pi, p.L,  \
                       p.KCAP, nq, p.nq_pad, dX, dY, (int)d, K, (refine && p.ksel > K) ? p.ksel : K, self_mode, self_offset, d_dist, d_idx, K, k0, kmax, \
                       d_w, d_fs, lnc, partial, qperm, p.part, p.nparts, qpb, border, nunits, col0, col1, p.pl_nr, \
                       refine ? reinterpret_cast<const double*>(ws + p.off_center) : nullptr)
    if (write_dist && !fuse) { if (refine) MCE_MERGE(true, false, true); else MCE_MERGE(true, false, false); }
    else if (write_dist && fuse) { if (refine) MCE_MERGE(true, true, true); else MCE_MERGE(true, true, false); }
    else { if (refine) MCE_MERGE(false, true, true); else MCE_MERGE(false, true, false); }
#undef MCE_MERGE
    MCE_HIP(hipGetLastError());
    return MCE_OK;
}

int finish_dotp(const double* partial, int64_t ncols, int k0, int kmax, double* d_dotp, hipStream_t st)
{
    const unsigned blocks = (unsigned)std::max<int64_t>((ncols + mce::kRedThreads - 1) / mce::kRedThreads, 1);
    hipLaunchKernelGGL(mce::dotp_final_kernel, dim3((unsigned)kmax), dim3(mce::kRedThreads), 0, st, partial, (int64_t)blocks, k0, kmax, d_dotp);
    MCE_HIP(hipGetLastError());
    return MCE_OK;
}
int zero_dotp(double* d_dotp, int kmax, hipStream_t st) { MCE_HIP(mce::zero_async(d_dotp, (size_t)kmax * sizeof(double), st)); return MCE_OK; }

}
```

### mcevidence_amd/csrc/knn_deep.hpp

```cpp
#pragma once
#include "knn_panel.hpp"

namespace mce {

struct DeepArgs {
    const _Float16* Yh;
    const _Float16* Xh;
    const double* qinfo;
    const double* params;
    const double* X;
    const double* Y;
    double* part_d;
    int* part_i;
    int64_t nq, nr, nq_pad, self_offset;
    int64_t nchunk_total;
    int D, ksel, self_exclude, nqblk, rsplit;
    int seed_tg;
    int debug;
    int seed_groups = 0;
    const double* lo_d = nullptr;
    const int* lo_i = nullptr;
};

__host__ __device__ constexpr int deep_chunk_tiles(int KST) { return KST == 5 ? 8 : (KST == 6 ? 8 : 6); }
constexpr int kDeepQueue = 448;
__host__ __device__ constexpr size_t deep_lds_bytes(int KST)
{
    return (size_t)2 * deep_chunk_tiles(KST) * KST * 1024
           + (size_t)kHWaves * kDeepQueue * 16
           + (size_t)kHWaves * kHQT * 32 * 4 + 128
           + (size_t)kHWaves * kHQT * 32 * 4
           + (size_t)kHWaves * deep_chunk_tiles(KST) * kHQT * 4;
}
__host__ __device__ constexpr bool deep_supported(int D, int K) { return D >= 64 && D <= 127 && K >= 1 && K <= 32; }
__host__ __device__ constexpr int deep_ksteps(int D) { return (D + 1 + 15) / 16 == 7 ? 8 : (D + 1 + 15) / 16; }

template <int KST, int KCAP, bool LOWER = false>
__global__ __launch_bounds__(kHThreads, 2) void knn_deep_kernel(DeepArgs a)
{
    static_assert(!LOWER || KCAP == 16, "second pass: 16-entry lists");
    static_assert(kHQT == 2 && (KST == 5 || KST == 6 || KST == 8), "8 waves x 2 query tiles; 5, 6 or 8 k-steps");
    constexpr int QT = 2;
    constexpr int QPW = 64;
    constexpr int QPB = kHWaves * QPW;
    constexpr int CT = deep_chunk_tiles(KST);
    constexpr int CHUNK_BYTES = CT * KST * 1024;
    constexpr int VPT = CHUNK_BYTES / 16 / kHThreads;
    static_assert(CHUNK_BYTES % (16 * kHThreads) == 0 && CT % 2 == 0, "chunk geometry");
    constexpr int QN = kDeepQueue;

    extern __shared__ __attribute__((aligned(16))) char lds_raw[];
    char* const stage0 = lds_raw;
    double* const qd2_all = reinterpret_cast<double*>(lds_raw + 2 * CHUNK_BYTES);
    int* const qpk_all = reinterpret_cast<int*>(qd2_all + kHWaves * QN);
    int* const qnx_all = qpk_all + kHWaves * QN;
    int* const head_all = qnx_all + kHWaves * QN;
    volatile int* const wvote = head_all + kHWaves * QPW;
    float* const sthr_all = reinterpret_cast<float*>(head_all + kHWaves * QPW + 32);
    int* const redo_all = reinterpret_cast<int*>(sthr_all + kHWaves * QPW);

    const int tid = threadIdx.x;
    const int lane = tid & 63;
    const int wave = __builtin_amdgcn_readfirstlane(tid >> 6);
    double* const wqd = qd2_all + wave * QN;
    int* const wq = qpk_all + wave * QN;
    int* const wnx = qnx_all + wave * QN;
    int* const whead = head_all + wave * QPW;
    float* const sthr = sthr_all + wave * QPW;
    int* const wredo = redo_all + wave * (CT * QT);
    const double INF = __builtin_huge_val();

    const int qblk = (int)(blockIdx.x % (unsigned)a.nqblk);
    const int split = (int)(blockIdx.x / (unsigned)a.nqblk);
    const int64_t c_lo = a.nchunk_total * split / a.rsplit, c_hi = a.nchunk_total * (split + 1) / a.rsplit;
    const int ntot = (int)(c_hi - c_lo);
    const int64_t qwave0 = (int64_t)qblk * QPB + wave * QPW;

    whead[lane] = -1;
    if (tid < 3) wvote[tid] = 0;

    double own_d[KCAP];
    int own_i[KCAP];
#pragma unroll
    for (int k = 0; k < KCAP; ++k) { own_d[k] = INF; own_i[k] = -1; }
    double lo_own_d = -1.0;
    int lo_own_i = -1;
    if constexpr (LOWER) {
        const int64_t o = ((int64_t)split * KCAP + (KCAP - 1)) * a.nq_pad + qwave0 + lane;
        lo_own_d = gptr(a.lo_d)[o];
        lo_own_i = gptr(a.lo_i)[o];
    }

    v8h b[QT][KST];
    float G[QT];
    unsigned lanew[QT];
    const int k_last = a.ksel - 1;
    {
        const auto Xh = gptr(a.Xh);
#pragma unroll
        for (int qt = 0; qt < QT; ++qt) {
            const int64_t q = qwave0 + qt * 32 + (lane & 31);
#pragma unroll
            for (int ks = 0; ks < KST; ++ks)
                b[qt][ks] = *(const __attribute__((address_space(1))) v8h*)(Xh + q * (int64_t)(16 * KST) + 16 * ks + 8 * (lane >> 5));
            lanew[qt] = ((unsigned)(qt * 32 + (lane & 31)) << kHRelBits) | (unsigned)(4 * (lane >> 5));
            G[qt] = -__builtin_huge_valf();
        }
    }
    double gq_a[QT], gq_c[QT], gq_xn[QT], gq_eps[QT], s2c;
    {
        const auto params = gptr(a.params);
        const auto qinfo = gptr(a.qinfo);
        const double p_scale = params[HP_SCALE], p_ey = params[HP_EY], p_ym = params[HP_YHATMAX], p_rho = params[HP_RHO];
        s2c = p_scale * p_scale;
#pragma unroll
        for (int qt = 0; qt < QT; ++qt) {
            const int64_t q = qwave0 + qt * 32 + (lane & 31);
            gq_a[qt] = 0.0;
            gq_c[qt] = -INF;
            gq_xn[qt] = 0.0;
            gq_eps[qt] = 0.0;
            if (q < a.nq) {
                const double xn = qinfo[2 * q + 1];
                const F16GateTerms t = f16_gate_terms(qinfo[2 * q], xn, p_ey, p_ym, p_rho, KST);
                gq_a[qt] = t.a;
                gq_c[qt] = t.c;
                gq_xn[qt] = xn;
                gq_eps[qt] = t.eps;
            }
        }
    }
    auto gate_of = [&](double thr, int qt) __attribute__((always_inline)) -> float { return f16_gate(thr, s2c, gq_a[qt], gq_c[qt]); };

    const int qlimit_gate = (a.debug & 8) ? -1 : QN - 64;
    int qcount = 0;
    int nredo = 0;
    double seed_thr = INF;

    auto drain = [&]() __attribute__((always_inline)) {
        const auto X = gptr(a.X);
        const auto Y = gptr(a.Y);
        const int D = a.D;
        const int64_t nq = a.nq, nr = a.nr;
        {
            const int sub = lane & 7;
            constexpr int EPL = 16;
            for (int b0 = 0; b0 < qcount; b0 += 8) {
                const int e = b0 + (lane >> 3);
                int ql = 0, j = 0;
                const bool valid = e < qcount;
                if (valid) {
                    const unsigned ent = (unsigned)wq[e];
                    ql = (int)(ent >> kHRelBits);
                    j = (int)(ent & ((1u << kHRelBits) - 1u));
                }
                const int64_t q = qwave0 + ql;
                const bool ok = valid && j < nr && q < nq && !(a.self_exclude && (int64_t)j == a.self_offset + q);
                const auto xp = X + (ok ? q : 0) * (int64_t)D;
                const auto yp = Y + (ok ? (int64_t)j : 0) * D;
                double xv[EPL], yv[EPL];
#pragma unroll
                for (int v = 0; v < EPL; ++v) {
                    const int iv = (sub + 8 * v < D) ? sub + 8 * v : sub;
                    xv[v] = xp[iv];
                    yv[v] = yp[iv];
                }
                double a0 = 0.0;
#pragma unroll
                for (int v = 0; v < EPL; ++v) {
                    const double t = (sub + 8 * v < D) ? xv[v] - yv[v] : 0.0;
                    a0 = fma(t, t, a0);
                }
                a0 += __shfl_xor(a0, 1, 64);
                a0 += __shfl_xor(a0, 2, 64);
                a0 += __shfl_xor(a0, 4, 64);
                if (sub == 0 && valid) {
                    wqd[e] = ok ? a0 : -1.0;
                    wq[e] = j;
                    if (ok && !(a0 > (double)sthr[ql])) wnx[e] = atomicExch(&whead[ql], e);
                }
            }
        }
        __builtin_amdgcn_fence(__ATOMIC_ACQ_REL, "wavefront");
        {
            int cur = whead[lane];
            whead[lane] = -1;
            while (__any(cur >= 0)) {
                const bool on = cur >= 0;
                const int ce = on ? cur : 0;
                double d2 = on ? wqd[ce] : INF;
                const int j = wq[ce];
                cur = on ? wnx[ce] : -1;
                if constexpr (LOWER) {
                    if (!(d2 > lo_own_d || (d2 == lo_own_d && j > lo_own_i))) d2 = INF;
                }
                list_insert<KCAP>(own_d, own_i, d2, j);
            }
        }
        qcount = 0;
        double thr_own = own_d[KCAP - 1];
#pragma unroll
        for (int k = 0; k < KCAP - 1; ++k) thr_own = (k == k_last) ? own_d[k] : thr_own;
        thr_own = fmin(thr_own, seed_thr);
        sthr[lane] = __double2float_ru(thr_own);
#pragma unroll
        for (int qt = 0; qt < QT; ++qt) G[qt] = gate_of(__shfl(thr_own, qt * 32 + (lane & 31), 64), qt);
    };

    auto event = [&](const v16f& c, const float (&l1)[5], const int qt, const float g, const int jb0, const unsigned todo, const int qlimit) __attribute__((always_inline)) -> unsigned {
        return f16_event<false>(c, l1, lanew[qt], g, false, jb0, todo, qlimit, wq, qcount);
    };

    const auto Yh_bytes = (const __attribute__((address_space(1))) char*)a.Yh;
    auto stage_async = [&](int64_t c, int buf) { f16_stage_chunk<VPT>(Yh_bytes + c * (int64_t)CHUNK_BYTES, stage0 + buf * CHUNK_BYTES, tid, wave); };
    auto tile_mfma = [&](const char* lp, v16f (&acc)[QT]) __attribute__((always_inline)) {
#pragma unroll
        for (int ks = 0; ks < KST; ++ks) {
            const v8h af = *reinterpret_cast<const v8h*>(lp + ks * 1024);
#pragma unroll
            for (int qt = 0; qt < QT; ++qt) {
                if (ks == 0) {
                    v16f z = {0.f, 0.f, 0.f, 0.f, 0.f, 0.f, 0.f, 0.f, 0.f, 0.f, 0.f, 0.f, 0.f, 0.f, 0.f, 0.f};
                    acc[qt] = __builtin_amdgcn_mfma_f32_32x32x16_f16(af, b[qt][0], z, 0, 0, 0);
                } else {
                    acc[qt] = __builtin_amdgcn_mfma_f32_32x32x16_f16(af, b[qt][ks], acc[qt], 0, 0, 0);
                }
            }
        }
#if defined(__HIP_DEVICE_COMPILE__)
        asm volatile("s_nop 15\n\ts_nop 3" : "+v"(acc[0]), "+v"(acc[1]));
#endif
    };

    stage_async(c_lo, 0);

    const int seed_G = a.seed_groups > 0 ? a.seed_groups : a.ksel + (a.self_exclude ? 1 : 0);
    const int seed_tiles = a.seed_tg > 0 ? seed_G * a.seed_tg : 0;
    if (seed_tiles > 0) {
        float gmax[QT] = {-__builtin_huge_valf(), -__builtin_huge_valf()};
        float gmin[QT] = {__builtin_huge_valf(), __builtin_huge_valf()};
        int in_group = 0;
        const int nchunks_seed = (seed_tiles + CT - 1) / CT;
        for (int k = 0; k < nchunks_seed; ++k) {
            const int buf = k & 1;
            dma_barrier();
            stage_async(k + 1 < nchunks_seed ? c_lo + k + 1 : c_lo, buf ^ 1);
            const char* const lbuf = stage0 + buf * CHUNK_BYTES + lane * 16;
            const int thi = seed_tiles - k * CT < CT ? seed_tiles - k * CT : CT;
            for (int t = 0; t < thi; ++t) {
                v16f acc[QT];
                tile_mfma(lbuf + (t * KST) * 1024, acc);
#pragma unroll
                for (int qt = 0; qt < QT; ++qt) {
                    float l1[5];
                    gmin[qt] = fminf(gmin[qt], f16_min16(acc[qt], l1));
                }
                if (++in_group == a.seed_tg) {
#pragma unroll
                    for (int qt = 0; qt < QT; ++qt) {
                        const float m = fminf(gmin[qt], __shfl_xor(gmin[qt], 32, 64));
                        gmax[qt] = fmaxf(gmax[qt], m);
                        gmin[qt] = __builtin_huge_valf();
                    }
                    in_group = 0;
                }
            }
        }
        double thr_q[QT];
#pragma unroll
        for (int qt = 0; qt < QT; ++qt) {
            thr_q[qt] = INF;
            if (gq_c[qt] > -INF && gmax[qt] < __builtin_huge_valf()) thr_q[qt] = f16_seed_bound((double)gmax[qt], gq_xn[qt], gq_eps[qt], gq_a[qt], s2c);
        }
        const double t_lo = __shfl(thr_q[0], lane & 31, 64), t_hi = __shfl(thr_q[1], lane & 31, 64);
        seed_thr = lane < 32 ? t_lo : t_hi;
        sthr[lane] = __double2float_ru(seed_thr);
#pragma unroll
        for (int qt = 0; qt < QT; ++qt) G[qt] = gate_of(thr_q[qt], qt);
    } else {
        sthr[lane] = __builtin_huge_valf();
#pragma unroll
        for (int qt = 0; qt < QT; ++qt) G[qt] = gate_of(INF, qt);
    }

    for (int k = 0; k < ntot; ++k) {
        const int buf = (seed_tiles > 0 ? ((seed_tiles + CT - 1) / CT + k) : k) & 1;
        const int64_t c = c_lo + k;
        const int vs = k % 3;
        if (qcount >= MCE_PANEL_TRIGGER && lane == 0) wvote[vs] = 1;
        dma_barrier();
        if (tid == 0) wvote[vs == 0 ? 2 : vs - 1] = 0;
        if (k + 1 < ntot) stage_async(c + 1, buf ^ 1);
        bool need_drain = __builtin_amdgcn_readfirstlane(wvote[vs]) != 0 || k + 1 == ntot;
        const char* const lbuf = stage0 + buf * CHUNK_BYTES + lane * 16;
        const int jchunk = (int)(c * (CT * 32));
        for (int t = 0; t < CT; ++t) {
            v16f acc[QT];
            tile_mfma(lbuf + (t * KST) * 1024, acc);
            float l1[QT][5], mm[QT];
            bool pq[QT];
#pragma unroll
            for (int qt = 0; qt < QT; ++qt) {
                mm[qt] = f16_min16(acc[qt], l1[qt]);
                pq[qt] = mm[qt] <= G[qt];
            }
            if (__any(pq[0] || pq[1])) {
#pragma unroll
                for (int qt = 0; qt < QT; ++qt) {
                    if (!__any(pq[qt])) continue;
                    const unsigned rem = event(acc[qt], l1[qt], qt, G[qt], jchunk + t * 32, 0xffffu, qlimit_gate);
                    if (rem) {
                        if (lane == 0) wredo[nredo] = (int)(rem | ((unsigned)qt << 16) | ((unsigned)t << 17));
                        nredo += 1;
                    }
                }
            }
        }
        while (need_drain || nredo > 0 || (k + 1 == ntot && qcount > 0)) {
            drain();
            need_drain = false;
            const int n = nredo;
            nredo = 0;
            for (int i = 0; i < n; ++i) {
                const unsigned w = (unsigned)__builtin_amdgcn_readfirstlane(wredo[i]);
                const unsigned todo = w & 0xffffu;
                const int qt = (int)((w >> 16) & 1u), t = (int)(w >> 17);
                v16f acc[QT];
                tile_mfma(lbuf + (t * KST) * 1024, acc);
                float l1[5];
                unsigned rem = 0;
                if (qt == 0) {
                    const float mm = f16_min16(acc[0], l1);
                    if (__any(mm <= G[0])) rem = event(acc[0], l1, 0, G[0], jchunk + t * 32, todo, QN - 64);
                } else {
                    const float mm = f16_min16(acc[1], l1);
                    if (__any(mm <= G[1])) rem = event(acc[1], l1, 1, G[1], jchunk + t * 32, todo, QN - 64);
                }
                if (rem) {
                    if (lane == 0) wredo[nredo] = (int)(rem | ((unsigned)qt << 16) | ((unsigned)t << 17));
                    nredo += 1;
                }
            }
        }
    }

    {
        const int64_t q = qwave0 + lane;
        const int64_t np = a.nq_pad;
        const auto pd = gptr_w(a.part_d) + (int64_t)split * KCAP * np;
        const auto pi = gptr_w(a.part_i) + (int64_t)split * KCAP * np;
#pragma unroll
        for (int k = 0; k < KCAP; ++k) {
            pd[(int64_t)k * np + q] = own_d[k];
            pi[(int64_t)k * np + q] = own_i[k];
        }
    }
}

}
```

### mcevidence_amd/csrc/knn_dispatch.hpp

```cpp
#pragma once
#include <hip/hip_runtime.h>
#include <stdint.h>

#include "sym_types.hpp"

namespace mce {

constexpr int kMaxDevices = 64;

struct KnnArgs {
    const double* Yf;
    int64_t nchunk_total;
    int rsplit;
    const double* X;
    const double* center;
    int64_t nq;
    int D;
    int64_t nq_pad;
    int nqblk;
    int self_exclude;
    int64_t self_offset;
    int ksel;
    double* part_d;
    int* part_i;
};

typedef hipError_t (*knn_launch_fn)(const KnnArgs&, hipStream_t);

struct KnnVariant {
    knn_launch_fn launch;
    int ks, kcap, qt, ct;
    size_t lds_bytes;
    const char* name;
};

struct KnnF16Args {
    const void* Yh;
    int64_t nchunk_total;
    int rsplit;
    const void* Xh;
    const double* qinfo;
    const double* params;
    const double* X;
    const double* Y;
    int64_t nq, nr;
    int D;
    int64_t nq_pad;
    int nqblk;
    int self_exclude;
    int64_t self_offset;
    int ksel;
    double* part_d;
    int* part_i;
    const int* clist = nullptr;
    const float* cdist = nullptr;
    int list_len = 0;
    const int* rperm = nullptr;
    const int* qperm = nullptr;
    const float* tbox_r = nullptr;
    const float* tbox_q = nullptr;
    const float* cbox_r = nullptr;
    const double* lo_d = nullptr;
    const int* lo_i = nullptr;
    int seed_cfg = 0;
    const int* border = nullptr;
    int qblk0 = 0, qblk_stride = 1, nqblk_run = 0;
    SymParams sym;
    float* wg_us = nullptr;
};
typedef hipError_t (*knn_f16_launch_fn)(const KnnF16Args&, hipStream_t);
struct PanelArgs;
typedef hipError_t (*knn_panel_launch_fn)(const PanelArgs&, hipStream_t);
struct KnnF16Variant {
    knn_f16_launch_fn launch;
    knn_f16_launch_fn launch_prune;
    knn_f16_launch_fn launch_lower;
    knn_f16_launch_fn launch_sym_pre;
    knn_f16_launch_fn launch_sym;
    knn_f16_launch_fn launch_sym_repair;
    knn_panel_launch_fn launch_panel;
    size_t lds_bytes_panel;
    size_t lds_bytes_sym;
    int kst, kcap, qt, ct;
    size_t lds_bytes;
    const char* name;
    knn_f16_launch_fn launch_prune_short;
    int prune_short_lc;
    knn_f16_launch_fn launch_prune_short2;
    int prune_short_lc2;
    knn_f16_launch_fn launch_wide;
    size_t lds_bytes_wide;
    knn_panel_launch_fn launch_panel_lower;
    knn_f16_launch_fn launch_sym_repair_lower;
    knn_f16_launch_fn launch_sym_pre32;
};
struct DeepArgs;
typedef hipError_t (*knn_deep_launch_fn)(const DeepArgs&, hipStream_t);
struct KnnDeepVariant {
    knn_deep_launch_fn launch;
    int kst, kcap, ct;
    size_t lds_bytes;
    const char* name;
    knn_deep_launch_fn launch_lower;
};
struct LongArgs;
typedef hipError_t (*knn_long_launch_fn)(const LongArgs&, hipStream_t);
struct KnnLongVariant {
    knn_long_launch_fn launch;
    int kcap, ct;
    size_t lds_bytes;
    const char* name;
};
constexpr int kNumLongKcap = 3;
extern const KnnLongVariant g_knn_long[kNumLongKcap];
constexpr int kNumDeepKST = 3;
extern const KnnDeepVariant g_knn_deep_kcap4[kNumDeepKST];
extern const KnnDeepVariant g_knn_deep_kcap8[kNumDeepKST];
extern const KnnDeepVariant g_knn_deep_kcap12[kNumDeepKST];
extern const KnnDeepVariant g_knn_deep_kcap16[kNumDeepKST];

constexpr int kMaxKST = 4;
extern const KnnF16Variant g_knn_f16_kcap4[kMaxKST];
extern const KnnF16Variant g_knn_f16_kcap8[kMaxKST];
extern const KnnF16Variant g_knn_f16_kcap12[kMaxKST];
extern const KnnF16Variant g_knn_f16_kcap16[kMaxKST];

constexpr int kMaxKS = 20;
constexpr int kWideMaxDim = 127;
__host__ __device__ constexpr int mfma_ks_for(int d) { return d <= 63 ? (d + 1 + 3) / 4 : ((d + 1 + 15) / 16) * 4; }
__host__ __device__ constexpr int mfma_variant_index(int KS) { return KS <= 16 ? KS - 1 : 11 + KS / 4; }
constexpr int kNumKcap = 6;
constexpr int kKcapList[kNumKcap] = {4, 8, 12, 16, 24, 32};

extern const KnnVariant g_knn_kcap4[kMaxKS];
extern const KnnVariant g_knn_kcap8[kMaxKS];
extern const KnnVariant g_knn_kcap12[kMaxKS];
extern const KnnVariant g_knn_kcap16[kMaxKS];
extern const KnnVariant g_knn_kcap24[kMaxKS];
extern const KnnVariant g_knn_kcap32[kMaxKS];

}
```

### mcevidence_amd/csrc/knn_inst.hip

```cpp
#include "knn_mfma.hpp"
#include "knn_f16.hpp"
#include "knn_panel.hpp"
#include "knn_deep.hpp"
#include "knn_dispatch.hpp"

#ifndef MCE_KCAP
#error "compile with -DMCE_KCAP=n"
#endif
#ifndef MCE_INST_PART
#define MCE_INST_PART 0
#endif
#define MCE_INST_F16 (MCE_KCAP <= 16 && (MCE_INST_PART == 0 || MCE_INST_PART == 1))
#define MCE_INST_F64 (MCE_INST_PART == 0 || MCE_INST_PART == 2)
#define MCE_INST_PANEL (MCE_KCAP <= 16 && (MCE_INST_PART == 0 || MCE_INST_PART == 3))
#define MCE_INST_DEEP (MCE_KCAP <= 16 && (MCE_INST_PART == 0 || MCE_INST_PART == 4))

namespace mce {

#if MCE_INST_F64
template <int KS, int KCAP>
hipError_t launch_variant(const KnnArgs& a, hipStream_t st)
{
    constexpr size_t LDS = lds_bytes(KS, KCAP);
    static_assert(LDS <= 160 * 1024, "LDS budget");
    static bool attr_set[kMaxDevices] = {};
    auto kern = knn_mfma_kernel<KS, KCAP>;
    int dev = 0;
    (void)hipGetDevice(&dev);
    if (dev >= kMaxDevices || !attr_set[dev]) {
        hipError_t e = hipFuncSetAttribute(reinterpret_cast<const void*>(kern), hipFuncAttributeMaxDynamicSharedMemorySize, (int)LDS);
        if (e != hipSuccess) return e;
        if (dev < kMaxDevices) attr_set[dev] = true;
    }
    const dim3 grid((unsigned)(a.nqblk * a.rsplit));
    hipLaunchKernelGGL(kern, grid, dim3(kThreads), LDS, st, a.Yf, a.nchunk_total, a.rsplit, a.X, a.center, a.nq, a.D,
                       a.nq_pad, a.nqblk, a.self_exclude, a.self_offset, a.ksel, a.part_d, a.part_i);
    return hipGetLastError();
}
#endif

#if MCE_INST_F16
template <int KST, int KCAP, bool PRUNE, bool LOWER = false, int SYM = 0, int LC = KCAP, int QTT = kHQT>
hipError_t launch_f16_variant(const KnnF16Args& a, hipStream_t st)
{
    constexpr size_t LDS_MAX = PRUNE ? f16_prune_lds_bytes(KST, 16 * KST - 1, LC) : f16_lds_bytes(KST, KCAP, SYM >= 2, QTT);
    static_assert(LDS_MAX <= 160 * 1024, "LDS budget");
    const size_t LDS = PRUNE ? f16_prune_lds_bytes(KST, a.D, LC) : LDS_MAX;
    static bool attr_set[kMaxDevices] = {};
    auto kern = knn_f16_kernel<KST, KCAP, PRUNE, LOWER, SYM, LC, QTT>;
    constexpr int WB = QTT / kHQT;
    int dev = 0;
    (void)hipGetDevice(&dev);
    if (dev >= kMaxDevices || !attr_set[dev]) {
        hipError_t e = hipFuncSetAttribute(reinterpret_cast<const void*>(kern), hipFuncAttributeMaxDynamicSharedMemorySize, (int)LDS_MAX);
        if (e != hipSuccess) return e;
        if (dev < kMaxDevices) attr_set[dev] = true;
    }
    const int ntiles_even = (int)((a.nr + 31) / 32) + (int)(((a.nr + 31) / 32) & 1);
    const int hv_n = PRUNE ? (a.seed_cfg & 0xffffff) : 0, hv_S = PRUNE && ((a.seed_cfg >> 24) & 0x7f) > 1 ? ((a.seed_cfg >> 24) & 0x7f) : 1;
    const dim3 grid((unsigned)(PRUNE ? (a.nqblk_run ? a.nqblk_run : a.nqblk * kHWaves) + hv_n * (hv_S - 1)
                               : SYM == 2 ? sym_unit_count(a.nqblk, kHWaves * kHQT, a.sym.panel * f16_chunk_tiles(KST), ntiles_even)
                               : SYM == 1 ? (a.nqblk_run ? a.nqblk_run : a.nqblk) : (a.nqblk / WB) * a.rsplit));
    hipLaunchKernelGGL(kern, grid, dim3(PRUNE ? 64 : kHThreads), LDS, st, static_cast<const _Float16*>(a.Yh), a.nchunk_total, a.rsplit,
                       static_cast<const _Float16*>(a.Xh), a.qinfo, a.params, a.X, a.Y, a.nq, a.nr, a.D, a.nq_pad, a.nqblk / WB,
                       a.self_exclude, a.self_offset, a.ksel, a.part_d, a.part_i, a.clist, a.cdist, a.list_len, a.rperm, a.qperm, a.tbox_r, a.tbox_q, a.cbox_r, a.qblk0, a.qblk_stride, a.border, a.lo_d, a.lo_i, a.seed_cfg, a.sym, a.wg_us);
    return hipGetLastError();
}
#endif

#if MCE_INST_F16 || MCE_INST_PANEL
template <int KST, int KCAP, bool LOWER = false>
hipError_t launch_panel_variant(const PanelArgs& a, hipStream_t st)
#if MCE_INST_PANEL
{
    constexpr size_t LDS = panel_lds_bytes(KST);
    static_assert(LDS <= 160 * 1024, "LDS budget");
    static bool attr_set[kMaxDevices] = {};
    auto kern = knn_panel_kernel<KST, KCAP, LOWER>;
    int dev = 0;
    (void)hipGetDevice(&dev);
    if (dev >= kMaxDevices || !attr_set[dev]) {
        hipError_t e = hipFuncSetAttribute(reinterpret_cast<const void*>(kern), hipFuncAttributeMaxDynamicSharedMemorySize, (int)LDS);
        if (e != hipSuccess) return e;
        if (dev < kMaxDevices) attr_set[dev] = true;
    }
    const int units = panel_unit_count(a.geom);
    if (units <= 0) return hipSuccess;
    hipLaunchKernelGGL(kern, dim3((unsigned)units), dim3(kHThreads), LDS, st, a);
    return hipGetLastError();
}
template hipError_t launch_panel_variant<1, MCE_KCAP>(const PanelArgs&, hipStream_t);
template hipError_t launch_panel_variant<2, MCE_KCAP>(const PanelArgs&, hipStream_t);
template hipError_t launch_panel_variant<3, MCE_KCAP>(const PanelArgs&, hipStream_t);
template hipError_t launch_panel_variant<4, MCE_KCAP>(const PanelArgs&, hipStream_t);
#if MCE_KCAP == 16
template hipError_t launch_panel_variant<1, MCE_KCAP, true>(const PanelArgs&, hipStream_t);
template hipError_t launch_panel_variant<2, MCE_KCAP, true>(const PanelArgs&, hipStream_t);
template hipError_t launch_panel_variant<3, MCE_KCAP, true>(const PanelArgs&, hipStream_t);
template hipError_t launch_panel_variant<4, MCE_KCAP, true>(const PanelArgs&, hipStream_t);
#endif
#else
;
extern template hipError_t launch_panel_variant<1, MCE_KCAP>(const PanelArgs&, hipStream_t);
extern template hipError_t launch_panel_variant<2, MCE_KCAP>(const PanelArgs&, hipStream_t);
extern template hipError_t launch_panel_variant<3, MCE_KCAP>(const PanelArgs&, hipStream_t);
extern template hipError_t launch_panel_variant<4, MCE_KCAP>(const PanelArgs&, hipStream_t);
#if MCE_KCAP == 16
extern template hipError_t launch_panel_variant<1, MCE_KCAP, true>(const PanelArgs&, hipStream_t);
extern template hipError_t launch_panel_variant<2, MCE_KCAP, true>(const PanelArgs&, hipStream_t);
extern template hipError_t launch_panel_variant<3, MCE_KCAP, true>(const PanelArgs&, hipStream_t);
extern template hipError_t launch_panel_variant<4, MCE_KCAP, true>(const PanelArgs&, hipStream_t);
#endif
#endif
#endif

#if MCE_INST_DEEP
template <int KST, int KCAP, bool LOWER = false>
hipError_t launch_deep_variant(const DeepArgs& a, hipStream_t st)
{
    constexpr size_t LDS = deep_lds_bytes(KST);
    static_assert(LDS <= 160 * 1024, "LDS budget");
    static bool attr_set[kMaxDevices] = {};
    auto kern = knn_deep_kernel<KST, KCAP, LOWER>;
    int dev = 0;
    (void)hipGetDevice(&dev);
    if (dev >= kMaxDevices || !attr_set[dev]) {
        hipError_t e = hipFuncSetAttribute(reinterpret_cast<const void*>(kern), hipFuncAttributeMaxDynamicSharedMemorySize, (int)LDS);
        if (e != hipSuccess) return e;
        if (dev < kMaxDevices) attr_set[dev] = true;
    }
    hipLaunchKernelGGL(kern, dim3((unsigned)(a.nqblk * a.rsplit)), dim3(kHThreads), LDS, st, a);
    return hipGetLastError();
}
#endif

#define MCE_STR2(x) #x
#define MCE_STR(x) MCE_STR2(x)
#define MCE_VARIANT(KS)                                                                                  \
    {&launch_variant<KS, MCE_KCAP>, KS, MCE_KCAP, mfma_qt(KS), chunk_tiles(KS, MCE_KCAP), lds_bytes(KS, MCE_KCAP),  \
     "knn_mfma_kernel<KS=" #KS ",KCAP=" MCE_STR(MCE_KCAP) ">"}

#define MCE_CAT2(a, b) a##b
#define MCE_CAT(a, b) MCE_CAT2(a, b)

#if !defined(__HIP_DEVICE_COMPILE__)
#if MCE_INST_F64
extern const KnnVariant MCE_CAT(g_knn_kcap, MCE_KCAP)[kMaxKS] = {
    MCE_VARIANT(1),  MCE_VARIANT(2),  MCE_VARIANT(3),  MCE_VARIANT(4),  MCE_VARIANT(5),  MCE_VARIANT(6),
    MCE_VARIANT(7),  MCE_VARIANT(8),  MCE_VARIANT(9),  MCE_VARIANT(10), MCE_VARIANT(11), MCE_VARIANT(12),
    MCE_VARIANT(13), MCE_VARIANT(14), MCE_VARIANT(15), MCE_VARIANT(16),
    MCE_VARIANT(20), MCE_VARIANT(24), MCE_VARIANT(28), MCE_VARIANT(32),
};
#endif
#if MCE_INST_F16
#if MCE_KCAP == 16
#define MCE_F16_LOWER(KST) (&launch_f16_variant<KST, MCE_KCAP, false, true>)
#define MCE_F16_SYM_LOWER(KST) &launch_panel_variant<KST, MCE_KCAP, true>, &launch_f16_variant<KST, MCE_KCAP, false, true, 3>, &launch_f16_variant<KST, 32, false, false, 1>
#else
#define MCE_F16_LOWER(KST) nullptr
#define MCE_F16_SYM_LOWER(KST) nullptr, nullptr, nullptr
#endif
#if MCE_KCAP == 12
#define MCE_F16_SHORT(KST) ((KST) == 1 ? &launch_f16_variant<1, MCE_KCAP, true, false, 0, 9> : (knn_f16_launch_fn) nullptr), ((KST) == 1 ? 9 : 0), \
                           ((KST) == 1 ? &launch_f16_variant<1, MCE_KCAP, true, false, 0, 10> : (knn_f16_launch_fn) nullptr), ((KST) == 1 ? 10 : 0)
#else
#define MCE_F16_SHORT(KST) nullptr, 0, nullptr, 0
#endif
#if MCE_KCAP == 4
#define MCE_F16_WIDE(KST) ((KST) == 1 ? &launch_f16_variant<1, MCE_KCAP, false, false, 0, MCE_KCAP, 4> : (knn_f16_launch_fn) nullptr), ((KST) == 1 ? f16_lds_bytes(1, MCE_KCAP, false, 4) : 0)
#else
#define MCE_F16_WIDE(KST) nullptr, 0
#endif
#define MCE_F16_VARIANT(KST, PRUNE_FN)                                                                   \
    {&launch_f16_variant<KST, MCE_KCAP, false>, PRUNE_FN, MCE_F16_LOWER(KST), &launch_f16_variant<KST, MCE_KCAP, false, false, 1>, \
     &launch_f16_variant<KST, MCE_KCAP, false, false, 2>, &launch_f16_variant<KST, MCE_KCAP, false, false, 3>, &launch_panel_variant<KST, MCE_KCAP>, panel_lds_bytes(KST), \
     f16_lds_bytes(KST, MCE_KCAP, true), KST, MCE_KCAP, f16_qt(MCE_KCAP), f16_chunk_tiles(KST), \
     f16_lds_bytes(KST, MCE_KCAP), "knn_f16_kernel<KST=" #KST ",KCAP=" MCE_STR(MCE_KCAP) ">", MCE_F16_SHORT(KST), MCE_F16_WIDE(KST), MCE_F16_SYM_LOWER(KST)}
extern const KnnF16Variant MCE_CAT(g_knn_f16_kcap, MCE_KCAP)[kMaxKST] = {
    MCE_F16_VARIANT(1, (&launch_f16_variant<1, MCE_KCAP, true>)), MCE_F16_VARIANT(2, nullptr), MCE_F16_VARIANT(3, nullptr),
    MCE_F16_VARIANT(4, nullptr),
};
#endif
#if MCE_INST_DEEP
#if MCE_KCAP == 16
#define MCE_DEEP_LOWER(KST) (&launch_deep_variant<KST, MCE_KCAP, true>)
#else
#define MCE_DEEP_LOWER(KST) nullptr
#endif
#define MCE_DEEP_VARIANT(KST) {&launch_deep_variant<KST, MCE_KCAP>, KST, MCE_KCAP, deep_chunk_tiles(KST), deep_lds_bytes(KST), "knn_deep_kernel<KST=" #KST ",KCAP=" MCE_STR(MCE_KCAP) ">", MCE_DEEP_LOWER(KST)}
extern const KnnDeepVariant MCE_CAT(g_knn_deep_kcap, MCE_KCAP)[kNumDeepKST] = {MCE_DEEP_VARIANT(5), MCE_DEEP_VARIANT(6), MCE_DEEP_VARIANT(8)};
#endif
#else
#if MCE_INST_DEEP
template __global__ void knn_deep_kernel<5, MCE_KCAP>(DeepArgs);
template __global__ void knn_deep_kernel<6, MCE_KCAP>(DeepArgs);
template __global__ void knn_deep_kernel<8, MCE_KCAP>(DeepArgs);
#if MCE_KCAP == 16
template __global__ void knn_deep_kernel<5, MCE_KCAP, true>(DeepArgs);
template __global__ void knn_deep_kernel<6, MCE_KCAP, true>(DeepArgs);
template __global__ void knn_deep_kernel<8, MCE_KCAP, true>(DeepArgs);
#endif
#endif
#if MCE_INST_F16
#define MCE_F16_INST(KST, PR, LW, SY) template __global__ void knn_f16_kernel<KST, MCE_KCAP, PR, LW, SY>(const _Float16*, int64_t, int, const _Float16*, const double*, const double*, const double*, const double*, int64_t, int64_t, int, int64_t, int, int, int64_t, int, double*, int*, const int*, const float*, int, const int*, const int*, const float*, const float*, const float*, int, int, const int*, const double*, const int*, int, SymParams, float*);
MCE_F16_INST(1, false, false, 0) MCE_F16_INST(2, false, false, 0) MCE_F16_INST(3, false, false, 0) MCE_F16_INST(4, false, false, 0) MCE_F16_INST(1, true, false, 0)
MCE_F16_INST(1, false, false, 1) MCE_F16_INST(2, false, false, 1) MCE_F16_INST(3, false, false, 1) MCE_F16_INST(4, false, false, 1)
MCE_F16_INST(1, false, false, 2) MCE_F16_INST(2, false, false, 2) MCE_F16_INST(3, false, false, 2) MCE_F16_INST(4, false, false, 2)
MCE_F16_INST(1, false, false, 3) MCE_F16_INST(2, false, false, 3) MCE_F16_INST(3, false, false, 3) MCE_F16_INST(4, false, false, 3)
#if MCE_KCAP == 12
template __global__ void knn_f16_kernel<1, MCE_KCAP, true, false, 0, 9>(const _Float16*, int64_t, int, const _Float16*, const double*, const double*, const double*, const double*, int64_t, int64_t, int, int64_t, int, int, int64_t, int, double*, int*, const int*, const float*, int, const int*, const int*, const float*, const float*, const float*, int, int, const int*, const double*, const int*, int, SymParams, float*);
template __global__ void knn_f16_kernel<1, MCE_KCAP, true, false, 0, 10>(const _Float16*, int64_t, int, const _Float16*, const double*, const double*, const double*, const double*, int64_t, int64_t, int, int64_t, int, int, int64_t, int, double*, int*, const int*, const float*, int, const int*, const int*, const float*, const float*, const float*, int, int, const int*, const double*, const int*, int, SymParams, float*);
#endif
#if MCE_KCAP == 16
MCE_F16_INST(1, false, true, 0) MCE_F16_INST(2, false, true, 0) MCE_F16_INST(3, false, true, 0) MCE_F16_INST(4, false, true, 0)
MCE_F16_INST(1, false, true, 3) MCE_F16_INST(2, false, true, 3) MCE_F16_INST(3, false, true, 3) MCE_F16_INST(4, false, true, 3)
#define MCE_F16_INST32(KST) template __global__ void knn_f16_kernel<KST, 32, false, false, 1>(const _Float16*, int64_t, int, const _Float16*, const double*, const double*, const double*, const double*, int64_t, int64_t, int, int64_t, int, int, int64_t, int, double*, int*, const int*, const float*, int, const int*, const int*, const float*, const float*, const float*, int, int, const int*, const double*, const int*, int, SymParams, float*);
MCE_F16_INST32(1) MCE_F16_INST32(2) MCE_F16_INST32(3) MCE_F16_INST32(4)
#endif
#if MCE_KCAP == 4
template __global__ void knn_f16_kernel<1, MCE_KCAP, false, false, 0, MCE_KCAP, 4>(const _Float16*, int64_t, int, const _Float16*, const double*, const double*, const double*, const double*, int64_t, int64_t, int, int64_t, int, int, int64_t, int, double*, int*, const int*, const float*, int, const int*, const int*, const float*, const float*, const float*, int, int, const int*, const double*, const int*, int, SymParams, float*);
#endif
#endif
#if MCE_INST_PANEL
template __global__ void knn_panel_kernel<1, MCE_KCAP>(PanelArgs);
template __global__ void knn_panel_kernel<2, MCE_KCAP>(PanelArgs);
template __global__ void knn_panel_kernel<3, MCE_KCAP>(PanelArgs);
template __global__ void knn_panel_kernel<4, MCE_KCAP>(PanelArgs);
#if MCE_KCAP == 16
template __global__ void knn_panel_kernel<1, MCE_KCAP, true>(PanelArgs);
template __global__ void knn_panel_kernel<2, MCE_KCAP, true>(PanelArgs);
template __global__ void knn_panel_kernel<3, MCE_KCAP, true>(PanelArgs);
template __global__ void knn_panel_kernel<4, MCE_KCAP, true>(PanelArgs);
#endif
#endif
#if MCE_INST_F64
#define MCE_INST(KS) template __global__ void knn_mfma_kernel<KS, MCE_KCAP>(const double*, int64_t, int, const double*, const double*, int64_t, int, int64_t, int, int, int64_t, int, double*, int*);
MCE_INST(1) MCE_INST(2) MCE_INST(3) MCE_INST(4) MCE_INST(5) MCE_INST(6) MCE_INST(7) MCE_INST(8)
MCE_INST(9) MCE_INST(10) MCE_INST(11) MCE_INST(12) MCE_INST(13) MCE_INST(14) MCE_INST(15) MCE_INST(16)
MCE_INST(20) MCE_INST(24) MCE_INST(28) MCE_INST(32)
#endif
#endif

}
```

### mcevidence_amd/csrc/knn_panel.hpp

```cpp
#pragma once
#include "knn_f16.hpp"

namespace mce {

struct PanelArgs {
    const _Float16* Yh;
    const _Float16* Xh;
    const double* qinfo;
    const double* params;
    const double* X;
    const double* Y;
    const int* rperm;
    double* part_d;
    int* part_i;
    int64_t nq, nr, nq_pad, self_offset;
    int D, ksel, self_exclude, spin_limit;
    int debug;
    SymParams sym;
    PanelGeom geom;
    const PanelUnit* units = nullptr;
    const double* lo_d = nullptr;
    const int* lo_i = nullptr;
};

#ifndef MCE_PANEL_STATS
#define MCE_PANEL_STATS 0
#endif
#ifndef MCE_PANEL_NPASS
#define MCE_PANEL_NPASS 3
#endif
#ifndef MCE_PANEL_STAGE_KB
#define MCE_PANEL_STAGE_KB MCE_H_STAGE_KB
#endif
#ifndef MCE_PANEL_QUEUE
#define MCE_PANEL_QUEUE MCE_H_QUEUE
#endif
#ifndef MCE_PANEL_TRIGGER
#define MCE_PANEL_TRIGGER 192
#endif
#ifndef MCE_PANEL_ABL
#define MCE_PANEL_ABL 0
#endif

__host__ __device__ constexpr int panel_chunk_tiles(int KST) { return MCE_PANEL_STAGE_KB / KST / 2 * 2; }
constexpr int kPanelQueue = MCE_PANEL_QUEUE;
__host__ __device__ constexpr size_t panel_lds_bytes(int KST)
{
    return (size_t)2 * panel_chunk_tiles(KST) * KST * 1024
           + (size_t)kHWaves * kPanelQueue * 16
           + (size_t)kHWaves * kHQT * 32 * 4 + 128
           + (size_t)kHWaves * kHQT * 32 * 4
           + (size_t)kHWaves * panel_chunk_tiles(KST) * kHQT * 4;
}

template <class T> __device__ __forceinline__ const __attribute__((address_space(1))) T* gptr(const T* p)
{
    return (const __attribute__((address_space(1))) T*)p;
}
template <class T> __device__ __forceinline__ __attribute__((address_space(1))) T* gptr_w(T* p)
{
    return (__attribute__((address_space(1))) T*)p;
}

__device__ __forceinline__ float vmaxf(float a, float b)
{
    float r;
    asm("v_max_f32 %0, %1, %2" : "=v"(r) : "v"(a), "v"(b));
    return r;
}

template <int KST, int KCAP, bool LOWER = false>
__global__ __launch_bounds__(kHThreads, 2) void knn_panel_kernel(PanelArgs args_by_value)
{
    static_assert(kHQT == 2 && kHNL == 1, "8 waves x 2 query tiles, one list per owner lane");
    constexpr int QT = 2;
    constexpr int QPW = 64;
    constexpr int QPB = kHWaves * QPW;
    constexpr int TPB = QPB / 32;
    constexpr int CT = panel_chunk_tiles(KST);
    constexpr int CHUNK_BYTES = CT * KST * 1024;
    constexpr int VPT = CHUNK_BYTES / 16 / kHThreads;
    static_assert(CHUNK_BYTES % (16 * kHThreads) == 0 && CT % 2 == 0, "chunk geometry");
    constexpr int QN = kPanelQueue;
    (void)args_by_value;
    typedef const __attribute__((address_space(4))) PanelArgs* ArgsPtr;
    const ArgsPtr ap0 = (ArgsPtr)__builtin_amdgcn_kernarg_segment_ptr();
#define MCE_ARGS() ([&]() __attribute__((always_inline)) { ArgsPtr p_ = ap0; asm volatile("" : "+s"(p_)); return p_; }())

    extern __shared__ __attribute__((aligned(16))) char lds_raw[];
    char* const stage0 = lds_raw;
    double* const qd2_all = reinterpret_cast<double*>(lds_raw + 2 * CHUNK_BYTES);
    int* const qpk_all = reinterpret_cast<int*>(qd2_all + kHWaves * QN);
    int* const qnx_all = qpk_all + kHWaves * QN;
    int* const head_all = qnx_all + kHWaves * QN;
    volatile int* const wvote = head_all + kHWaves * QPW;
    float* const sthr_all = reinterpret_cast<float*>(head_all + kHWaves * QPW + 32);
    int* const redo_all = reinterpret_cast<int*>(sthr_all + kHWaves * QPW);

    const int tid = threadIdx.x;
    const int lane = tid & 63;
    const int wave = __builtin_amdgcn_readfirstlane(tid >> 6);
    double* const wqd = qd2_all + wave * QN;
    int* const wq = qpk_all + wave * QN;
    int* const wnx = qnx_all + wave * QN;
    int* const whead = head_all + wave * QPW;
    float* const sthr = sthr_all + wave * QPW;
    int* const wredo = redo_all + wave * (CT * QT);
    const double INF = __builtin_huge_val();

#if MCE_PANEL_STATS
    const long long t_kernel0 = clock64();
    long long st_drains = 0, st_enq = 0, st_events = 0, st_redo = 0, st_tD = 0, st_tE = 0, st_tPro = 0, st_tA = 0, st_tR = 0, st_tB = 0;
#endif

    int sym_p, qblk, t_lo, t_hi, useq, sym_on, qb_lo;
    {
        const ArgsPtr a = MCE_ARGS();
        if (a->units) {
            const auto u = (const __attribute__((address_space(1))) PanelUnit*)a->units + blockIdx.x;
            qblk = __builtin_amdgcn_readfirstlane(u->qblk);
            t_lo = __builtin_amdgcn_readfirstlane(u->t_lo);
            t_hi = __builtin_amdgcn_readfirstlane(u->t_hi);
            useq = __builtin_amdgcn_readfirstlane(u->useq);
            sym_p = 0;
            sym_on = a->geom.sym_on;
            qb_lo = a->geom.qb_lo;
        } else {
            PanelGeom g;
            g.qb_lo = a->geom.qb_lo; g.qb_hi = a->geom.qb_hi; g.tpb = a->geom.tpb; g.tpp = a->geom.tpp;
            g.ct = a->geom.ct; g.ntiles = a->geom.ntiles; g.sym_on = a->geom.sym_on;
            panel_unit_decode((int)blockIdx.x, g, sym_p, qblk);
            panel_unit_tiles(sym_p, qblk, g, t_lo, t_hi);
            useq = panel_unit_seq(sym_p, qblk, g);
            sym_on = g.sym_on;
            qb_lo = g.qb_lo;
        }
    }
    auto chain_of = [&](int& chain, int64_t& list_off) __attribute__((always_inline)) {
        const ArgsPtr a = MCE_ARGS();
        chain = qblk;
        list_off = 0;
        if (a->units) {
            const auto u = (const __attribute__((address_space(1))) PanelUnit*)a->units + blockIdx.x;
            chain = __builtin_amdgcn_readfirstlane(u->chain);
            list_off = (int64_t)__builtin_amdgcn_readfirstlane(u->list_set) * KCAP * a->nq_pad;
        }
    };
    const int64_t qwave0 = (int64_t)qblk * QPB + wave * QPW;

    whead[lane] = -1;
    if (tid < 3) wvote[tid] = 0;

    double own_d[KCAP];
    int own_i[KCAP];
#pragma unroll
    for (int k = 0; k < KCAP; ++k) { own_d[k] = INF; own_i[k] = -1; }
    double seed_thr = INF;

    {
        const ArgsPtr a = MCE_ARGS();
        if (useq > 0) {
            int chain;
            int64_t list_off;
            chain_of(chain, list_off);
            int spins = 0;
            const int limit = ((a->debug & 16) && useq == 1 && (wave & 1)) ? -1 : a->spin_limit;
            bool ok = true;
            const auto done = gptr(a->sym.done);
            while (spins > limit || __hip_atomic_load(done + chain, __ATOMIC_RELAXED, __HIP_MEMORY_SCOPE_AGENT) < useq) {
                if (++spins > limit) { ok = false; break; }
                __builtin_amdgcn_s_sleep(32);
            }
            __builtin_amdgcn_fence(__ATOMIC_ACQUIRE, "agent");
            if (ok && gptr(a->sym.bucket_flag)[qblk] != 0) ok = false;
            if (ok) {
                const int64_t q = qwave0 + lane;
                const int64_t np = a->nq_pad;
                const auto pd = gptr(a->part_d) + list_off;
                const auto pi = gptr(a->part_i) + list_off;
#pragma unroll
                for (int k = 0; k < KCAP; ++k) {
                    own_d[k] = pd[(int64_t)k * np + q];
                    own_i[k] = pi[(int64_t)k * np + q];
                }
            } else if (lane == 0) {
                gptr_w(a->sym.bucket_flag)[qblk] = 1;
            }
        }
    }

    v8h b[QT][KST];
    float G[QT], cR[QT];
    unsigned lanew[QT];
    const int k_last = MCE_ARGS()->ksel - 1;
    {
        const ArgsPtr a = MCE_ARGS();
        const auto Xh = gptr(a->Xh);
#pragma unroll
        for (int qt = 0; qt < QT; ++qt) {
            const int64_t q = qwave0 + qt * 32 + (lane & 31);
#pragma unroll
            for (int ks = 0; ks < KST; ++ks)
                b[qt][ks] = *(const __attribute__((address_space(1))) v8h*)(Xh + q * (int64_t)(16 * KST) + 16 * ks + 8 * (lane >> 5));
            lanew[qt] = ((unsigned)(qt * 32 + (lane & 31)) << kHRelBits) | (unsigned)(4 * (lane >> 5));
            cR[qt] = -__builtin_huge_valf();
            G[qt] = -__builtin_huge_valf();
        }
    }
    double gq_a[QT], gq_c[QT], own_a = 0.0, s2c, rowc;
    {
        const ArgsPtr a = MCE_ARGS();
        const auto params = gptr(a->params);
        const auto qinfo = gptr(a->qinfo);
        const double p_scale = params[HP_SCALE], p_ey = params[HP_EY], p_ym = params[HP_YHATMAX], p_rho = params[HP_RHO];
        s2c = p_scale * p_scale;
        rowc = f16_row_const(p_ym);
#pragma unroll
        for (int qt = 0; qt < QT; ++qt) {
            const int64_t q = qwave0 + qt * 32 + (lane & 31);
            gq_a[qt] = 0.0;
            gq_c[qt] = -INF;
            if (q < a->nq && MCE_PANEL_ABL != 1) {
                const F16GateTerms t = f16_gate_terms(qinfo[2 * q], qinfo[2 * q + 1], p_ey, p_ym, p_rho, KST);
                gq_a[qt] = t.a;
                gq_c[qt] = t.c;
            }
        }
        {
            const int64_t q = qwave0 + lane;
            if (q < a->nq) own_a = f16_gate_a(qinfo[2 * q], p_ey, KST);
        }
    }
    auto gate_of = [&](double thr, int qt) __attribute__((always_inline)) -> float { return f16_gate(thr, s2c, gq_a[qt], gq_c[qt]); };
    auto own_row_gate = [&](double thr) __attribute__((always_inline)) -> float { return f16_row_gate(thr, s2c, own_a, rowc); };
    {
        const ArgsPtr a = MCE_ARGS();
        const int64_t q = qwave0 + lane;
        double t0 = INF;
        if (sym_on) t0 = __longlong_as_double((long long)__hip_atomic_load(gptr(a->sym.thr) + q, __ATOMIC_RELAXED, __HIP_MEMORY_SCOPE_AGENT));
        else if (a->sym.thr) t0 = __longlong_as_double((long long)gptr(a->sym.thr)[q]);
        seed_thr = t0;
        double tl = own_d[KCAP - 1];
#pragma unroll
        for (int k = 0; k < KCAP - 1; ++k) tl = (k == k_last) ? own_d[k] : tl;
        t0 = fmin(t0, tl);
        sthr[lane] = __double2float_ru(t0);
#pragma unroll
        for (int qt = 0; qt < QT; ++qt) G[qt] = gate_of(__shfl(t0, qt * 32 + (lane & 31), 64), qt);
        if (sym_on) {
#pragma unroll
            for (int qt = 0; qt < QT; ++qt) cR[qt] = gq_c[qt] > -INF ? f16_round_up(gq_c[qt]) : -__builtin_huge_valf();
        }
    }

    const int dbg_flags = MCE_ARGS()->debug;
    const int qlimit_gate = (dbg_flags & 8) ? -1 : QN - 64;
    int qcount = 0;
    int nredo = 0;

    auto drain = [&]() __attribute__((always_inline)) {
#if MCE_PANEL_STATS
        const long long t_d0 = clock64();
        st_drains += 1; st_enq += qcount;
#endif
        const ArgsPtr a = MCE_ARGS();
        const auto X = gptr(a->X);
        const auto Y = gptr(a->Y);
        const int D = a->D;
        const int64_t nq = a->nq, nr = a->nr;
        const int self_exclude = a->self_exclude;
        const int64_t self_offset = a->self_offset;
        const auto rperm = gptr(a->rperm);
        {
            const int sub = lane & 7;
            constexpr int NPASS = KST > 2 ? 1 : MCE_PANEL_NPASS;
            constexpr int EPL = KST > 2 ? 8 : 4;
            for (int b0 = 0; b0 < qcount; b0 += NPASS * 8) {
                int qlp[NPASS], ep[NPASS];
                bool okp[NPASS];
                const __attribute__((address_space(1))) double* xp[NPASS];
                const __attribute__((address_space(1))) double* yp[NPASS];
#pragma unroll
                for (int u = 0; u < NPASS; ++u) {
                    const int e = b0 + u * 8 + (lane >> 3);
                    ep[u] = e;
                    int ql = 0, j = 0;
                    const bool valid = e < qcount;
                    if (valid) {
                        const unsigned ent = (unsigned)wq[e];
                        ql = (int)(ent >> kHRelBits);
                        j = (int)(ent & ((1u << kHSymRowBits) - 1u));
                    }
                    qlp[u] = ql;
                    const int64_t q = qwave0 + ql;
                    okp[u] = valid && j < nr && q < nq && !(self_exclude && (int64_t)j == self_offset + q);
                    xp[u] = X + (okp[u] ? q : 0) * (int64_t)D;
                    yp[u] = Y + (okp[u] ? (int64_t)j : 0) * D;
                }
                double xv[NPASS][EPL], yv[NPASS][EPL];
#pragma unroll
                for (int u = 0; u < NPASS; ++u)
#pragma unroll
                    for (int v = 0; v < EPL; ++v) {
                        const int iv = (sub + 8 * v < D) ? sub + 8 * v : (sub < D ? sub : D - 1);
                        xv[u][v] = xp[u][iv];
                        yv[u][v] = yp[u][iv];
                    }
#pragma unroll
                for (int u = 0; u < NPASS; ++u) {
                    double a0 = 0.0;
#pragma unroll
                    for (int v = 0; v < EPL; ++v) {
                        const double t = (sub + 8 * v < D) ? xv[u][v] - yv[u][v] : 0.0;
                        a0 = fma(t, t, a0);
                    }
                    a0 += __shfl_xor(a0, 1, 64);
                    a0 += __shfl_xor(a0, 2, 64);
                    a0 += __shfl_xor(a0, 4, 64);
                    if (sub == 0 && ep[u] < qcount) {
                        wqd[ep[u]] = okp[u] ? a0 : -1.0;
                        bool col = okp[u] && !(a0 > (double)sthr[qlp[u]]);
                        if constexpr (LOWER) {
                            if (col) {
                                const int64_t o = (int64_t)(KCAP - 1) * a->nq_pad + qwave0 + qlp[u];
                                const double ld = gptr(a->lo_d)[o];
                                const int li = gptr(a->lo_i)[o];
                                const int jr = (int)((unsigned)wq[ep[u]] & ((1u << kHSymRowBits) - 1u));
                                const int jc = rperm ? rperm[jr] : jr;
                                col = a0 > ld || (a0 == ld && jc > li);
                            }
                        }
                        if (col) wnx[ep[u]] = atomicExch(&whead[qlp[u]], ep[u]);
                    }
                }
            }
        }
        __builtin_amdgcn_fence(__ATOMIC_ACQ_REL, "wavefront");
#if MCE_PANEL_STATS
        const long long t_dA = clock64();
        st_tA += t_dA - t_d0;
#endif
        {
            const auto sp_thr = gptr_w(a->sym.thr);
            const auto sp_rrow = gptr_w(a->sym.rrow);
            const auto sp_rtile = gptr_w(a->sym.rtile);
            const auto sp_slots = gptr_w(a->sym.slots);
            const auto sp_bucket_cnt = gptr_w(a->sym.bucket_cnt);
            const auto sp_bucket_flag = gptr_w(a->sym.bucket_flag);
            const auto sp_bucket = gptr_w(a->sym.bucket);
            const int sp_cap = a->sym.cap;
            const int ksel = a->ksel;
            auto row_gate = [&](double thr, int row) { return f16_row_gate_of(thr, gptr(a->qinfo)[2 * (int64_t)row], a->params, KST); };
            for (int e0 = 0; e0 < qcount; e0 += 64) {
                const int e = e0 + lane;
                const bool valid = e < qcount;
                const unsigned ent = valid ? (unsigned)wq[e] : 0u;
                const int ql = (int)(ent >> kHRelBits);
                const int j = (int)(ent & ((1u << kHSymRowBits) - 1u));
                const bool rowflag = (ent >> kHSymRowBits) & 1u;
                const double d2 = valid ? wqd[e] : -1.0;
                const bool ok = valid && d2 >= 0.0;
                const int oj = ok ? (rperm ? rperm[j] : j) : -1;
                bool rs = ok && rowflag;
                if (rs) {
                    const int jb = j / QPB;
                    rs = d2 <= __longlong_as_double((long long)__hip_atomic_load(sp_thr + j, __ATOMIC_RELAXED, __HIP_MEMORY_SCOPE_AGENT));
                    if constexpr (LOWER) {
                        if (rs) {
                            const int64_t o = (int64_t)(KCAP - 1) * a->nq_pad + j;
                            const double ld = gptr(a->lo_d)[o];
                            const int li = gptr(a->lo_i)[o];
                            const int sc = rperm ? rperm[qwave0 + ql] : (int)(qwave0 + ql);
                            rs = d2 > ld || (d2 == ld && sc > li);
                        }
                    }
                    if (rs) rs = sym_slot_insert<KCAP>(sp_slots, sp_thr, sp_rrow, sp_rtile, ksel, j, d2, row_gate);
                    if (rs) {
                        const int slot = __hip_atomic_fetch_add(sp_bucket_cnt + jb, 1, __ATOMIC_RELAXED, __HIP_MEMORY_SCOPE_AGENT);
                        if ((unsigned)slot < (unsigned)sp_cap) {
                            const auto en = sp_bucket + ((int64_t)jb * sp_cap + slot);
                            en->d2 = d2;
                            en->src = rperm ? rperm[qwave0 + ql] : (int)(qwave0 + ql);
                            en->row = j;
                        } else {
                            sp_bucket_flag[jb] = 1;
                        }
                    }
                }
                if (valid) wq[e] = oj;
            }
        }
        __builtin_amdgcn_fence(__ATOMIC_ACQ_REL, "wavefront");
#if MCE_PANEL_STATS
        const long long t_dR = clock64();
        st_tR += t_dR - t_dA;
#endif
        {
            int cur = whead[lane];
            whead[lane] = -1;
            while (__any(cur >= 0)) {
                const bool on = cur >= 0;
                const int ce = on ? cur : 0;
                const double d2 = on ? wqd[ce] : INF;
                const int j = wq[ce];
                cur = on ? wnx[ce] : -1;
                list_insert<KCAP>(own_d, own_i, d2, j);
            }
        }
        qcount = 0;
        double thr_own = own_d[KCAP - 1];
#pragma unroll
        for (int k = 0; k < KCAP - 1; ++k) thr_own = (k == k_last) ? own_d[k] : thr_own;
        thr_own = fmin(thr_own, seed_thr);
        if (sym_on) {
            const auto sp_thr = gptr_w(a->sym.thr);
            const auto sp_rrow = gptr_w(a->sym.rrow);
            const auto sp_rtile = gptr_w(a->sym.rtile);
            const int64_t q = qwave0 + lane;
            double t = thr_own;
            float R = 0.0f;
            if (q < nq) {
                if (t < INF) {
                    const unsigned long long mb = (unsigned long long)__double_as_longlong(t);
                    const unsigned rb = __float_as_uint(own_row_gate(t));
                    const unsigned long long ob = __hip_atomic_fetch_min(sp_thr + q, mb, __ATOMIC_RELAXED, __HIP_MEMORY_SCOPE_AGENT);
                    const unsigned orb = __hip_atomic_fetch_min(sp_rrow + q, rb, __ATOMIC_RELAXED, __HIP_MEMORY_SCOPE_AGENT);
                    t = fmin(t, __longlong_as_double((long long)ob));
                    R = __uint_as_float(rb < orb ? rb : orb);
                } else {
                    t = __longlong_as_double((long long)__hip_atomic_load(sp_thr + q, __ATOMIC_RELAXED, __HIP_MEMORY_SCOPE_AGENT));
                    const unsigned rb = __float_as_uint(own_row_gate(t));
                    const unsigned orb = __hip_atomic_fetch_min(sp_rrow + q, rb, __ATOMIC_RELAXED, __HIP_MEMORY_SCOPE_AGENT);
                    R = __uint_as_float(rb < orb ? rb : orb);
                }
            }
            thr_own = t;
            seed_thr = t;
            float m = R;
#pragma unroll
            for (int o = 16; o >= 1; o >>= 1) m = fmaxf(m, __shfl_xor(m, o, 64));
            if ((lane & 31) == 0) __hip_atomic_store(sp_rtile + ((qwave0 + lane) >> 5), m, __ATOMIC_RELAXED, __HIP_MEMORY_SCOPE_AGENT);
        }
        sthr[lane] = __double2float_ru(thr_own);
#pragma unroll
        for (int qt = 0; qt < QT; ++qt) G[qt] = gate_of(__shfl(thr_own, qt * 32 + (lane & 31), 64), qt);
#if MCE_PANEL_STATS
        st_tD += clock64() - t_d0;
#endif
    };

    auto event = [&](const v16f& c, const float (&l1)[5], const int qt, const float gq, const bool rowflag, const int jb0, const unsigned todo, const int qlimit) __attribute__((always_inline)) -> unsigned {
        return f16_event<true>(c, l1, lanew[qt], gq, rowflag, jb0, todo, qlimit, wq, qcount);
    };

    const auto Yh_bytes = (const __attribute__((address_space(1))) char*)MCE_ARGS()->Yh;
    auto stage_async = [&](int64_t c, int buf) { f16_stage_chunk<VPT>(Yh_bytes + c * (int64_t)CHUNK_BYTES, stage0 + buf * CHUNK_BYTES, tid, wave); };
    auto load_a = [&](const char* lp, v8h (&a)[KST]) { f16_load_a<KST>(lp, a); };
    auto mfma_first = [&](const v8h (&a)[KST], v16f (&acc)[QT]) __attribute__((always_inline)) {
#pragma unroll
        for (int qt = 0; qt < QT; ++qt) {
            v16f z = {0.f, 0.f, 0.f, 0.f, 0.f, 0.f, 0.f, 0.f, 0.f, 0.f, 0.f, 0.f, 0.f, 0.f, 0.f, 0.f};
            acc[qt] = __builtin_amdgcn_mfma_f32_32x32x16_f16(a[0], b[qt][0], z, 0, 0, 0);
        }
    };
    auto mfma_rest = [&](const v8h (&a)[KST], v16f (&acc)[QT]) __attribute__((always_inline)) {
#pragma unroll
        for (int ks = 1; ks < KST; ++ks)
#pragma unroll
            for (int qt = 0; qt < QT; ++qt) acc[qt] = __builtin_amdgcn_mfma_f32_32x32x16_f16(a[ks], b[qt][ks], acc[qt], 0, 0, 0);
    };
#if defined(__HIP_DEVICE_COMPILE__)
#define MCE_ORDER(GATED_, NEXT_) asm volatile("" : "+v"(GATED_[0]), "+v"(GATED_[1]), "+v"(NEXT_[0]), "+v"(NEXT_[1]))
#else
#define MCE_ORDER(GATED_, NEXT_) do {} while (0)
#endif
    auto gate_tile = [&](const v16f (&acc)[QT], const int jb0, const float (&gq)[QT], const float (&rg)[QT], const int tix) __attribute__((always_inline)) {
#if MCE_PANEL_ABL == 2
#if defined(__HIP_DEVICE_COMPILE__)
        asm volatile("" :: "v"(acc[0]), "v"(acc[1]));
#endif
        return;
#endif
        float l1[QT][5], mm[QT];
        bool pq[QT];
#pragma unroll
        for (int qt = 0; qt < QT; ++qt) {
            mm[qt] = f16_min16(acc[qt], l1[qt]);
            pq[qt] = mm[qt] <= gq[qt];
        }
        if (__any(pq[0] || pq[1])) {
#pragma unroll
            for (int qt = 0; qt < QT; ++qt) {
                if (!__any(pq[qt])) continue;
#if MCE_PANEL_STATS
                st_events += 1;
                const long long t_e0 = clock64();
#endif
                const unsigned rem = event(acc[qt], l1[qt], qt, gq[qt], mm[qt] <= rg[qt], jb0, 0xffffu, qlimit_gate);
                if (rem) {
                    if (lane == 0) wredo[nredo] = (int)(rem | ((unsigned)qt << 16) | ((unsigned)tix << 17));
                    nredo += 1;
                }
#if MCE_PANEL_STATS
                st_tE += clock64() - t_e0;
#endif
            }
        }
    };

    const int cfirst = t_lo / CT;
    const int ntot = (t_hi - 1) / CT - cfirst + 1;
    const auto rtile_p = gptr(MCE_ARGS()->sym.rtile);
    auto rt_load = [&](int c) -> float {
        const int t = c * CT + lane;
        const int tb = t / TPB;
        const bool en = sym_on && lane < CT && tb >= qb_lo && tb < qblk && MCE_PANEL_ABL != 1;
        const float r = en ? __hip_atomic_load(rtile_p + t, __ATOMIC_RELAXED, __HIP_MEMORY_SCOPE_AGENT) : -__builtin_huge_valf();
        return fmaxf(r, __shfl_xor(r, 1, 64));
    };
    float rt_cur = -__builtin_huge_valf(), rt_next;
    stage_async(cfirst, 0);
    rt_next = rt_load(cfirst);
#if MCE_PANEL_STATS
    st_tPro = clock64() - t_kernel0;
#endif
    v16f accA[QT], accB[QT];
    for (int k = 0; k < ntot; ++k) {
        const int buf = k & 1;
        const int c = cfirst + k;
        const int vs = k % 3;
        if (qcount >= MCE_PANEL_TRIGGER && lane == 0) wvote[vs] = 1;
#if MCE_PANEL_STATS
        const long long t_b0 = clock64();
#endif
        dma_barrier();
#if MCE_PANEL_STATS
        st_tB += clock64() - t_b0;
#endif
        if (tid == 0) wvote[vs == 0 ? 2 : vs - 1] = 0;
        rt_cur = rt_next;
        if (k + 1 < ntot) {
            stage_async(c + 1, buf ^ 1);
            rt_next = rt_load(c + 1);
        }
        bool need_drain = __builtin_amdgcn_readfirstlane(wvote[vs]) != 0 || k + 1 == ntot;
        const int tlo = (k == 0) ? t_lo - c * CT : 0;
        const int thi = t_hi - c * CT < CT ? t_hi - c * CT : CT;
        const char* const lbuf = stage0 + buf * CHUNK_BYTES + lane * 16;
        const int jchunk = c * (CT * 32);
        {
            v8h a0[KST], a1[KST];
            load_a(lbuf + (tlo * KST) * 1024, a0);
            load_a(lbuf + ((tlo + 1) * KST) * 1024, a1);
            mfma_first(a0, accA);
            mfma_rest(a0, accA);
            int t = tlo;
            float gqP[QT], rgP[QT];
            _Pragma("unroll 1") for (;;)
            {
                const float rP = __uint_as_float((unsigned)__builtin_amdgcn_readlane((int)__float_as_uint(rt_cur), t));
#pragma unroll
                for (int qt = 0; qt < QT; ++qt) {
                    rgP[qt] = rP + cR[qt];
                    gqP[qt] = vmaxf(G[qt], rgP[qt]);
                }
                const bool more = t + 2 < thi;
                load_a(lbuf + ((more ? t + 2 : t) * KST) * 1024, a0);
                mfma_first(a1, accB);
                MCE_ORDER(accA, accB);
                mfma_rest(a1, accB);
                gate_tile(accA, jchunk + t * 32, gqP, rgP, t);
                if (!more) break;
                load_a(lbuf + ((t + 3) * KST) * 1024, a1);
                mfma_first(a0, accA);
                MCE_ORDER(accB, accA);
                mfma_rest(a0, accA);
                gate_tile(accB, jchunk + (t + 1) * 32, gqP, rgP, t + 1);
                t += 2;
            }
            {
#if defined(__HIP_DEVICE_COMPILE__)
                asm volatile("s_nop 15\n\ts_nop 3" : "+v"(accB[0]), "+v"(accB[1]));
#endif
                gate_tile(accB, jchunk + (t + 1) * 32, gqP, rgP, t + 1);
            }
        }
        while (need_drain || nredo > 0 || (k + 1 == ntot && qcount > 0)) {
            drain();
            need_drain = false;
            const int n = nredo;
            nredo = 0;
            for (int i = 0; i < n; ++i) {
                const unsigned w = (unsigned)__builtin_amdgcn_readfirstlane(wredo[i]);
                const unsigned todo = w & 0xffffu;
                const int qt = (int)((w >> 16) & 1u), t = (int)(w >> 17);
                const float Rt = __uint_as_float((unsigned)__builtin_amdgcn_readlane((int)__float_as_uint(rt_cur), t));
                v8h at[KST];
                load_a(lbuf + (t * KST) * 1024, at);
                v16f z = {0.f, 0.f, 0.f, 0.f, 0.f, 0.f, 0.f, 0.f, 0.f, 0.f, 0.f, 0.f, 0.f, 0.f, 0.f, 0.f};
                v16f r_ = z;
                if (qt == 0) {
#pragma unroll
                    for (int ks = 0; ks < KST; ++ks) r_ = __builtin_amdgcn_mfma_f32_32x32x16_f16(at[ks], b[0][ks], r_, 0, 0, 0);
                } else {
#pragma unroll
                    for (int ks = 0; ks < KST; ++ks) r_ = __builtin_amdgcn_mfma_f32_32x32x16_f16(at[ks], b[1][ks], r_, 0, 0, 0);
                }
#if defined(__HIP_DEVICE_COMPILE__)
                asm volatile("s_nop 15\n\ts_nop 3" : "+v"(r_));
#endif
                float l1[5];
                const float mm = f16_min16(r_, l1);
                const float rg = Rt + (qt ? cR[1] : cR[0]);
                const float gq = vmaxf(qt ? G[1] : G[0], rg);
                unsigned rem = 0;
                if (__any(mm <= gq)) rem = event(r_, l1, qt, gq, mm <= rg, jchunk + t * 32, todo, QN - 64);
                if (rem) {
                    if (lane == 0) wredo[nredo] = (int)(rem | ((unsigned)qt << 16) | ((unsigned)t << 17));
                    nredo += 1;
                }
#if MCE_PANEL_STATS
                st_redo += 1;
#endif
            }
        }
    }

#if MCE_PANEL_STATS
    if (lane == 0) {
        const ArgsPtr a = MCE_ARGS();
        double* o = const_cast<double*>(a->params) + 16 + ((int64_t)blockIdx.x * kHWaves + wave) * 8;
        o[0] = (double)st_drains; o[1] = (double)st_enq; o[2] = (double)st_redo; o[3] = (double)st_events;
        o[4] = (double)st_tE; o[5] = (double)st_tD; o[6] = (double)(clock64() - t_kernel0); o[7] = (double)st_tPro;
        double* o2 = const_cast<double*>(a->params) + 16 + ((int64_t)gridDim.x * kHWaves) * 8 + ((int64_t)blockIdx.x * kHWaves + wave) * 8;
        o2[0] = (double)st_tA; o2[1] = (double)st_tR; o2[2] = (double)(st_tD - st_tA - st_tR); o2[3] = (double)st_tB; o2[4] = 0; o2[5] = 0; o2[6] = 0; o2[7] = 0;
    }
#endif
    {
        const ArgsPtr a = MCE_ARGS();
        const int64_t q = qwave0 + lane;
        const int64_t np = a->nq_pad;
        int chain;
        int64_t list_off;
        chain_of(chain, list_off);
        const auto pd = gptr_w(a->part_d) + list_off;
        const auto pi = gptr_w(a->part_i) + list_off;
#pragma unroll
        for (int k = 0; k < KCAP; ++k) {
            pd[(int64_t)k * np + q] = own_d[k];
            pi[(int64_t)k * np + q] = own_i[k];
        }
        __builtin_amdgcn_fence(__ATOMIC_RELEASE, "agent");
        __syncthreads();
        if (tid == 0) __hip_atomic_fetch_add(gptr_w(a->sym.done) + chain, 1, __ATOMIC_RELAXED, __HIP_MEMORY_SCOPE_AGENT);
    }
#undef MCE_ARGS
}

}
```

Measured before the change: 26.53 million.

## Reuse idle stage buffer as drain scratch, decouple panel chunk tiles and queue sizing

The panel kernel no longer keeps per-wave distance and next-pointer queue arrays in LDS. During a drain it borrows the idle half of the double-buffered stage, waiting for outstanding loads first and re-issuing the next stage load afterwards. The LDS this frees allows larger panel chunk tiles, a bigger queue and a per-KST trigger, with new panel-specific chunk constants, and reference packing is padded to a multiple of both tile widths. The cost is a serialized wait and reload of the next chunk whenever a drain happens, which exposes load latency.

```diff
diff --git a/mcevidence_amd/csrc/capi_apo.hpp b/mcevidence_amd/csrc/capi_apo.hpp
--- a/mcevidence_amd/csrc/capi_apo.hpp
+++ b/mcevidence_amd/csrc/capi_apo.hpp
@@ -27,8 +27,8 @@
     const int env_panel = env_pairs_once_panel();
     int S = std::min(8, std::max(1, (1536 + nown - 1) / std::max(nown, 1)));
     if (env_split) S = env_split;
-    const int def_panel = kSymPanelChunks[p.KST];
-    int panel = S > 1 ? (int)std::max<int64_t>(8, std::min<int64_t>(def_panel, p.nchunk / (2 * S))) : 0;
+    const int def_panel = kSymPanelChunksPanel[p.KST];
+    int panel = S > 1 ? (int)std::max<int64_t>(8, std::min<int64_t>(def_panel, p.nrow_pack / ((int64_t)p.PCT * 32) / (2 * S))) : 0;
     if (env_panel) panel = env_panel;
     sh.nsplit = S;
     sh.panel = panel;
diff --git a/mcevidence_amd/csrc/capi_common.hpp b/mcevidence_amd/csrc/capi_common.hpp
--- a/mcevidence_amd/csrc/capi_common.hpp
+++ b/mcevidence_amd/csrc/capi_common.hpp
@@ -135,6 +135,7 @@
     ~SameSetHint() { g_same_set_hint = prev; }
 };
 constexpr int kSymPanelChunks[5] = {0, 96, 256, 256, 256};
+constexpr int kSymPanelChunksPanel[5] = {0, 72, 192, 256, 192};
 int sym_bucket_per_row(int K)
 {
     const int b = read_tuning().sym_bucket;
diff --git a/mcevidence_amd/csrc/capi_plan.hpp b/mcevidence_amd/csrc/capi_plan.hpp
--- a/mcevidence_amd/csrc/capi_plan.hpp
+++ b/mcevidence_amd/csrc/capi_plan.hpp
@@ -34,6 +34,8 @@
     int KS = 0, KCAP = 0, QT = 0, CT = 0;
     int64_t nchunk = 0;
     int64_t nrow_pad = 0;
+    int PCT = 0;
+    int64_t nrow_pack = 0;
     int nqblk = 0;
     int64_t nq_pad = 0;
     int rsplit = 1;
@@ -201,6 +203,7 @@
             p.vh = &by_kcap(ki, mce::g_knn_f16_kcap4, mce::g_knn_f16_kcap8, mce::g_knn_f16_kcap12, mce::g_knn_f16_kcap16)[p.KST - 1];
             p.QT = p.vh->qt;
             p.CT = p.vh->ct;
+            p.PCT = p.vh->ct_panel;
         }
         p.v = nullptr;
         qpb = mce::f16_qpb(p.KCAP);
@@ -272,11 +275,23 @@
     auto layout = [&]() {
     p.L = p.twopass ? 2 * p.rsplit : p.rsplit;
 
+    if (f16 && (!p.twopass || p.vh->launch_panel_lower) && !p.prune && nq == nr && p.vh->launch_sym && p.nqblk >= 2 && p.nrow_pad <= ((int64_t)1 << mce::kHSymRowBits)) {
+        const int sm = eff_sym_mode();
+        p.sym = sm == 2 || (sm == 0 && p.nqblk >= kSymAutoMinBlocks[p.KST] * ((p.KST == 1 && p.KCAP == 16) ? 2 : 1));
+        if (g_same_set_hint == 0 || (g_same_set_hint < 0 && t_opt.same_set == 0)) p.sym = false;
+    }
+    p.nrow_pack = p.nrow_pad;
+    if (p.sym) {
+        int64_t both = (int64_t)p.CT * 32;
+        while (both % ((int64_t)p.PCT * 32)) both += (int64_t)p.CT * 32;
+        p.nrow_pack = (p.nrow_pad + both - 1) / both * both;
+    }
+
     size_t off = 0;
     p.off_yf = off;
     if (filt) {
         p.off_yh = off;
-        off = align_up(off + (size_t)p.nrow_pad * (size_t)(16 * p.KST) * 2, 256);
+        off = align_up(off + (size_t)p.nrow_pack * (size_t)(16 * p.KST) * 2, 256);
         p.off_xh = off;
         off = align_up(off + (size_t)p.nq_pad * (size_t)(16 * p.KST) * 2, 256);
         p.off_qinfo = off;
@@ -286,11 +301,6 @@
     } else {
         off = align_up(off + (size_t)p.nrow_pad * (size_t)(4 * p.KS) * sizeof(double), 256);
     }
-    if (f16 && (!p.twopass || p.vh->launch_panel_lower) && !p.prune && nq == nr && p.vh->launch_sym && p.nqblk >= 2 && p.nrow_pad <= ((int64_t)1 << mce::kHSymRowBits)) {
-        const int sm = eff_sym_mode();
-        p.sym = sm == 2 || (sm == 0 && p.nqblk >= kSymAutoMinBlocks[p.KST] * ((p.KST == 1 && p.KCAP == 16) ? 2 : 1));
-        if (g_same_set_hint == 0 || (g_same_set_hint < 0 && t_opt.same_set == 0)) p.sym = false;
-    }
     p.sym_nsplit = 1;
     p.sym_panel = 0;
     if (p.sym && !p.twopass) {
@@ -298,7 +308,7 @@
         int S = 1;
         if (tun.sym_chains >= 1) S = std::min(tun.sym_chains, kSymMaxChains);
         p.sym_nsplit = S;
-        if (S > 1) p.sym_panel = (int)std::max<int64_t>(8, std::min<int64_t>(kSymPanelChunks[p.KST], p.nchunk / (2 * S)));
+        if (S > 1) p.sym_panel = (int)std::max<int64_t>(8, std::min<int64_t>(kSymPanelChunksPanel[p.KST], p.nrow_pack / ((int64_t)p.PCT * 32) / (2 * S)));
     }
     const int l_alloc = std::max(p.L, p.sym_nsplit);
     p.off_pd = off;
diff --git a/mcevidence_amd/csrc/capi_search.hpp b/mcevidence_amd/csrc/capi_search.hpp
--- a/mcevidence_amd/csrc/capi_search.hpp
+++ b/mcevidence_amd/csrc/capi_search.hpp
@@ -244,10 +244,10 @@
     hipLaunchKernelGGL(mce::f16_scale_kernel, dim3(1), dim3(64), 0, st, box_y, separate_queries ? box_x : (const double*)nullptr, params);
     MCE_HIP(hipGetLastError());
     const int64_t rows_per_block = 4 * (64 / (2 * p.KST));
-    const int64_t pack_blocks = std::min<int64_t>((p.nrow_pad + rows_per_block - 1) / rows_per_block, 2048);
+    const int64_t pack_blocks = std::min<int64_t>((p.nrow_pack + rows_per_block - 1) / rows_per_block, 2048);
     const bool one_pass = f.sX == f.sY && nq == nr && p.nq_pad <= p.nrow_pad;
     hipLaunchKernelGGL(mce::f16_pack_refs_kernel, dim3((unsigned)pack_blocks), dim3(256), 0, st,
-                       f.sY, nr, (int)d, p.KST, p.nrow_pad, center, params, yh, one_pass ? xh : (_Float16*)nullptr, one_pass ? qinfo : (double*)nullptr,
+                       f.sY, nr, (int)d, p.KST, p.nrow_pack, center, params, yh, one_pass ? xh : (_Float16*)nullptr, one_pass ? qinfo : (double*)nullptr,
                        one_pass ? p.nq_pad : (int64_t)0);
     MCE_HIP(hipGetLastError());
     if (!one_pass) {
@@ -363,15 +363,17 @@
     const int qb_hi = p.nparts > 1 && !p.apo ? (int)((int64_t)p.nqblk * (p.part + 1) / p.nparts) : p.nqblk;
     p.sym_qb_lo = qb_lo; p.sym_qb_hi = qb_hi;
     const bool panel_kernel = !tun.sym_kernel_f16 || p.nparts > 1 || p.twopass;
+    const int sweep_ct = panel_kernel ? p.PCT : p.CT;
+    if (panel_kernel && tun.sym_panel <= 0) a.sym.panel = kSymPanelChunksPanel[p.KST];
     mce::PanelGeom geom;
-    geom.qb_lo = qb_lo; geom.qb_hi = qb_hi; geom.tpb = mce::kHWaves * mce::kHQT; geom.ct = p.CT; geom.tpp = a.sym.panel * p.CT; geom.sym_on = 1;
+    geom.qb_lo = qb_lo; geom.qb_hi = qb_hi; geom.tpb = mce::kHWaves * mce::kHQT; geom.ct = sweep_ct; geom.tpp = a.sym.panel * sweep_ct; geom.sym_on = 1;
     geom.ntiles = (int)((nr + 31) / 32) + (int)(((nr + 31) / 32) & 1);
     const bool apo = p.apo && p.nparts > 1 && !p.twopass && panel_kernel;
     const bool chains1 = !apo && p.nparts == 1 && panel_kernel && !p.twopass && p.sym_nsplit > 1;
     if (apo) { geom.blk_first = p.part; geom.blk_stride = p.nparts; }
     if (apo || chains1) {
         const int pn = apo ? p.apo_panel : p.sym_panel;
-        if (pn > 0 && (apo || tun.sym_panel <= 0)) { a.sym.panel = pn; geom.tpp = a.sym.panel * p.CT; }
+        if (pn > 0 && (apo || tun.sym_panel <= 0)) { a.sym.panel = pn; geom.tpp = a.sym.panel * sweep_ct; }
         geom.nsplit = std::max(1, apo ? p.apo_nsplit : p.sym_nsplit);
         if (geom.nsplit > 1) {
             a.sym.done = reinterpret_cast<int*>(sw + p.sl.keys_b);
@@ -446,7 +448,7 @@
     g_last_flops_all = g_last_flops_main + (double)(seed_used & 0xffff) * p.CT * (double)(qb_hi - qb_lo) * 16.0 * 1024.0 * 32.0 * p.KST;
     snprintf(g_last_kernel, sizeof(g_last_kernel), "%s symmetric%s%s%s grid=%d block=%d lds=%zu qt=%d ct=%d panel=%d seed=%dx%d/%d bucket=%d", p.vh->name, panel_kernel ? " panel-kernel" : "",
              p.twopass ? " two passes" : "", geom.blk_stride > 1 ? " pairs-once" : (geom.nsplit > 1 ? " chains" : ""), sym_units,
-             mce::kHThreads, panel_kernel ? p.vh->lds_bytes_panel : p.vh->lds_bytes_sym, p.QT, p.CT, a.sym.panel, seed_used & 0xffff, (seed_used >> 16) & 0xfff, (seed_used >> 28) & 3, p.sl.cap);
+             mce::kHThreads, panel_kernel ? p.vh->lds_bytes_panel : p.vh->lds_bytes_sym, p.QT, sweep_ct, a.sym.panel, seed_used & 0xffff, (seed_used >> 16) & 0xfff, (seed_used >> 28) & 3, p.sl.cap);
     return MCE_OK;
 }
 
diff --git a/mcevidence_amd/csrc/knn_deep.hpp b/mcevidence_amd/csrc/knn_deep.hpp
--- a/mcevidence_amd/csrc/knn_deep.hpp
+++ b/mcevidence_amd/csrc/knn_deep.hpp
@@ -24,6 +24,7 @@
 
 __host__ __device__ constexpr int deep_chunk_tiles(int KST) { return KST == 5 ? 8 : (KST == 6 ? 8 : 6); }
 constexpr int kDeepQueue = 448;
+constexpr int kDeepTrigger = 192;
 __host__ __device__ constexpr size_t deep_lds_bytes(int KST)
 {
     return (size_t)2 * deep_chunk_tiles(KST) * KST * 1024
@@ -287,7 +288,7 @@
         const int buf = (seed_tiles > 0 ? ((seed_tiles + CT - 1) / CT + k) : k) & 1;
         const int64_t c = c_lo + k;
         const int vs = k % 3;
-        if (qcount >= MCE_PANEL_TRIGGER && lane == 0) wvote[vs] = 1;
+        if (qcount >= kDeepTrigger && lane == 0) wvote[vs] = 1;
         dma_barrier();
         if (tid == 0) wvote[vs == 0 ? 2 : vs - 1] = 0;
         if (k + 1 < ntot) stage_async(c + 1, buf ^ 1);
diff --git a/mcevidence_amd/csrc/knn_dispatch.hpp b/mcevidence_amd/csrc/knn_dispatch.hpp
--- a/mcevidence_amd/csrc/knn_dispatch.hpp
+++ b/mcevidence_amd/csrc/knn_dispatch.hpp
@@ -93,6 +93,7 @@
     knn_panel_launch_fn launch_panel_lower;
     knn_f16_launch_fn launch_sym_repair_lower;
     knn_f16_launch_fn launch_sym_pre32;
+    int ct_panel;
 };
 struct DeepArgs;
 typedef hipError_t (*knn_deep_launch_fn)(const DeepArgs&, hipStream_t);
diff --git a/mcevidence_amd/csrc/knn_inst.hip b/mcevidence_amd/csrc/knn_inst.hip
--- a/mcevidence_amd/csrc/knn_inst.hip
+++ b/mcevidence_amd/csrc/knn_inst.hip
@@ -175,7 +175,7 @@
     {&launch_f16_variant<KST, MCE_KCAP, false>, PRUNE_FN, MCE_F16_LOWER(KST), &launch_f16_variant<KST, MCE_KCAP, false, false, 1>, \
      &launch_f16_variant<KST, MCE_KCAP, false, false, 2>, &launch_f16_variant<KST, MCE_KCAP, false, false, 3>, &launch_panel_variant<KST, MCE_KCAP>, panel_lds_bytes(KST), \
      f16_lds_bytes(KST, MCE_KCAP, true), KST, MCE_KCAP, f16_qt(MCE_KCAP), f16_chunk_tiles(KST), \
-     f16_lds_bytes(KST, MCE_KCAP), "knn_f16_kernel<KST=" #KST ",KCAP=" MCE_STR(MCE_KCAP) ">", MCE_F16_SHORT(KST), MCE_F16_WIDE(KST), MCE_F16_SYM_LOWER(KST)}
+     f16_lds_bytes(KST, MCE_KCAP), "knn_f16_kernel<KST=" #KST ",KCAP=" MCE_STR(MCE_KCAP) ">", MCE_F16_SHORT(KST), MCE_F16_WIDE(KST), MCE_F16_SYM_LOWER(KST), panel_chunk_tiles(KST)}
 extern const KnnF16Variant MCE_CAT(g_knn_f16_kcap, MCE_KCAP)[kMaxKST] = {
     MCE_F16_VARIANT(1, (&launch_f16_variant<1, MCE_KCAP, true>)), MCE_F16_VARIANT(2, nullptr), MCE_F16_VARIANT(3, nullptr),
     MCE_F16_VARIANT(4, nullptr),
diff --git a/mcevidence_amd/csrc/knn_panel.hpp b/mcevidence_amd/csrc/knn_panel.hpp
--- a/mcevidence_amd/csrc/knn_panel.hpp
+++ b/mcevidence_amd/csrc/knn_panel.hpp
@@ -1,5 +1,6 @@
 #pragma once
 #include "knn_f16.hpp"
+#include "panel_geom.hpp"
 
 namespace mce {
 
@@ -29,29 +30,11 @@
 #ifndef MCE_PANEL_NPASS
 #define MCE_PANEL_NPASS 3
 #endif
-#ifndef MCE_PANEL_STAGE_KB
-#define MCE_PANEL_STAGE_KB MCE_H_STAGE_KB
-#endif
-#ifndef MCE_PANEL_QUEUE
-#define MCE_PANEL_QUEUE MCE_H_QUEUE
-#endif
-#ifndef MCE_PANEL_TRIGGER
-#define MCE_PANEL_TRIGGER 192
-#endif
 #ifndef MCE_PANEL_ABL
 #define MCE_PANEL_ABL 0
 #endif
 
-__host__ __device__ constexpr int panel_chunk_tiles(int KST) { return MCE_PANEL_STAGE_KB / KST / 2 * 2; }
-constexpr int kPanelQueue = MCE_PANEL_QUEUE;
-__host__ __device__ constexpr size_t panel_lds_bytes(int KST)
-{
-    return (size_t)2 * panel_chunk_tiles(KST) * KST * 1024
-           + (size_t)kHWaves * kPanelQueue * 16
-           + (size_t)kHWaves * kHQT * 32 * 4 + 128
-           + (size_t)kHWaves * kHQT * 32 * 4
-           + (size_t)kHWaves * panel_chunk_tiles(KST) * kHQT * 4;
-}
+static_assert(kPanelWaves == kHWaves && kPanelPieceStride == kHThreads * 16 && kHQT == 2, "panel_geom.hpp restates the workgroup geometry");
 
 template <class T> __device__ __forceinline__ const __attribute__((address_space(1))) T* gptr(const T* p)
 {
@@ -80,8 +63,12 @@
     constexpr int CT = panel_chunk_tiles(KST);
     constexpr int CHUNK_BYTES = CT * KST * 1024;
     constexpr int VPT = CHUNK_BYTES / 16 / kHThreads;
-    static_assert(CHUNK_BYTES % (16 * kHThreads) == 0 && CT % 2 == 0, "chunk geometry");
-    constexpr int QN = kPanelQueue;
+    static_assert(CHUNK_BYTES % (16 * kHThreads) == 0 && CT % 2 == 0 && CT <= 64, "chunk geometry");
+    constexpr int QN = panel_queue(KST);
+    constexpr int TRIGGER = panel_trigger(KST);
+    static_assert(panel_lds_bytes(KST) <= 160 * 1024, "LDS budget");
+    static_assert(VPT == panel_wave_pieces(KST) && QN * kPanelScratchEntryBytes <= VPT * kPanelPieceBytes, "drain scratch: 12 B x entries <= VPT KB");
+    static_assert(QN % 64 == 0 && TRIGGER > 0 && TRIGGER <= QN - 64, "queue geometry");
     (void)args_by_value;
     typedef const __attribute__((address_space(4))) PanelArgs* ArgsPtr;
     const ArgsPtr ap0 = (ArgsPtr)__builtin_amdgcn_kernarg_segment_ptr();
@@ -89,10 +76,8 @@
 
     extern __shared__ __attribute__((aligned(16))) char lds_raw[];
     char* const stage0 = lds_raw;
-    double* const qd2_all = reinterpret_cast<double*>(lds_raw + 2 * CHUNK_BYTES);
-    int* const qpk_all = reinterpret_cast<int*>(qd2_all + kHWaves * QN);
-    int* const qnx_all = qpk_all + kHWaves * QN;
-    int* const head_all = qnx_all + kHWaves * QN;
+    int* const qpk_all = reinterpret_cast<int*>(lds_raw + 2 * CHUNK_BYTES);
+    int* const head_all = qpk_all + kHWaves * QN;
     volatile int* const wvote = head_all + kHWaves * QPW;
     float* const sthr_all = reinterpret_cast<float*>(head_all + kHWaves * QPW + 32);
     int* const redo_all = reinterpret_cast<int*>(sthr_all + kHWaves * QPW);
@@ -100,9 +85,7 @@
     const int tid = threadIdx.x;
     const int lane = tid & 63;
     const int wave = __builtin_amdgcn_readfirstlane(tid >> 6);
-    double* const wqd = qd2_all + wave * QN;
     int* const wq = qpk_all + wave * QN;
-    int* const wnx = qnx_all + wave * QN;
     int* const whead = head_all + wave * QPW;
     float* const sthr = sthr_all + wave * QPW;
     int* const wredo = redo_all + wave * (CT * QT);
@@ -110,7 +93,7 @@
 
 #if MCE_PANEL_STATS
     const long long t_kernel0 = clock64();
-    long long st_drains = 0, st_enq = 0, st_events = 0, st_redo = 0, st_tD = 0, st_tE = 0, st_tPro = 0, st_tA = 0, st_tR = 0, st_tB = 0;
+    long long st_drains = 0, st_enq = 0, st_events = 0, st_redo = 0, st_tD = 0, st_tE = 0, st_tPro = 0, st_tA = 0, st_tR = 0, st_tB = 0, st_tW = 0, st_tS = 0, st_ends = 0;
 #endif
 
     int sym_p, qblk, t_lo, t_hi, useq, sym_on, qb_lo;
@@ -258,7 +241,9 @@
     int qcount = 0;
     int nredo = 0;
 
-    auto drain = [&]() __attribute__((always_inline)) {
+    auto drain = [&](char* const scr) __attribute__((always_inline)) {
+        auto wqd = [&](int e) __attribute__((always_inline)) -> double& { return *reinterpret_cast<double*>(scr + panel_scratch_offset(0, e, 0, QN)); };
+        auto wnx = [&](int e) __attribute__((always_inline)) -> int& { return *reinterpret_cast<int*>(scr + panel_scratch_offset(0, e, 1, QN)); };
 #if MCE_PANEL_STATS
         const long long t_d0 = clock64();
         st_drains += 1; st_enq += qcount;
@@ -318,7 +303,7 @@
                     a0 += __shfl_xor(a0, 2, 64);
                     a0 += __shfl_xor(a0, 4, 64);
                     if (sub == 0 && ep[u] < qcount) {
-                        wqd[ep[u]] = okp[u] ? a0 : -1.0;
+                        wqd(ep[u]) = okp[u] ? a0 : -1.0;
                         bool col = okp[u] && !(a0 > (double)sthr[qlp[u]]);
                         if constexpr (LOWER) {
                             if (col) {
@@ -330,7 +315,7 @@
                                 col = a0 > ld || (a0 == ld && jc > li);
                             }
                         }
-                        if (col) wnx[ep[u]] = atomicExch(&whead[qlp[u]], ep[u]);
+                        if (col) wnx(ep[u]) = atomicExch(&whead[qlp[u]], ep[u]);
                     }
                 }
             }
@@ -358,7 +343,7 @@
                 const int ql = (int)(ent >> kHRelBits);
                 const int j = (int)(ent & ((1u << kHSymRowBits) - 1u));
                 const bool rowflag = (ent >> kHSymRowBits) & 1u;
-                const double d2 = valid ? wqd[e] : -1.0;
+                const double d2 = valid ? wqd(e) : -1.0;
                 const bool ok = valid && d2 >= 0.0;
                 const int oj = ok ? (rperm ? rperm[j] : j) : -1;
                 bool rs = ok && rowflag;
@@ -401,9 +386,9 @@
             while (__any(cur >= 0)) {
                 const bool on = cur >= 0;
                 const int ce = on ? cur : 0;
-                const double d2 = on ? wqd[ce] : INF;
+                const double d2 = on ? wqd(ce) : INF;
                 const int j = wq[ce];
-                cur = on ? wnx[ce] : -1;
+                cur = on ? wnx(ce) : -1;
                 list_insert<KCAP>(own_d, own_i, d2, j);
             }
         }
@@ -515,9 +500,9 @@
         const int t = c * CT + lane;
         const int tb = t / TPB;
         const bool en = sym_on && lane < CT && tb >= qb_lo && tb < qblk && MCE_PANEL_ABL != 1;
-        const float r = en ? __hip_atomic_load(rtile_p + t, __ATOMIC_RELAXED, __HIP_MEMORY_SCOPE_AGENT) : -__builtin_huge_valf();
-        return fmaxf(r, __shfl_xor(r, 1, 64));
+        return en ? __hip_atomic_load(rtile_p + t, __ATOMIC_RELAXED, __HIP_MEMORY_SCOPE_AGENT) : -__builtin_huge_valf();
     };
+    auto rt_pair = [&](float r) -> float { return fmaxf(r, __shfl_xor(r, 1, 64)); };
     float rt_cur = -__builtin_huge_valf(), rt_next;
     stage_async(cfirst, 0);
     rt_next = rt_load(cfirst);
@@ -529,7 +514,7 @@
         const int buf = k & 1;
         const int c = cfirst + k;
         const int vs = k % 3;
-        if (qcount >= MCE_PANEL_TRIGGER && lane == 0) wvote[vs] = 1;
+        if (qcount >= TRIGGER && lane == 0) wvote[vs] = 1;
 #if MCE_PANEL_STATS
         const long long t_b0 = clock64();
 #endif
@@ -538,12 +523,12 @@
         st_tB += clock64() - t_b0;
 #endif
         if (tid == 0) wvote[vs == 0 ? 2 : vs - 1] = 0;
-        rt_cur = rt_next;
+        rt_cur = rt_pair(rt_next);
         if (k + 1 < ntot) {
             stage_async(c + 1, buf ^ 1);
             rt_next = rt_load(c + 1);
         }
-        bool need_drain = __builtin_amdgcn_readfirstlane(wvote[vs]) != 0 || k + 1 == ntot;
+        bool need_drain = __builtin_amdgcn_readfirstlane(*(volatile __attribute__((address_space(3))) int*)(wvote + vs)) != 0 || k + 1 == ntot;
         const int tlo = (k == 0) ? t_lo - c * CT : 0;
         const int thi = t_hi - c * CT < CT ? t_hi - c * CT : CT;
         const char* const lbuf = stage0 + buf * CHUNK_BYTES + lane * 16;
@@ -585,8 +570,19 @@
                 gate_tile(accB, jchunk + (t + 1) * 32, gqP, rgP, t + 1);
             }
         }
+        char* const scr = stage0 + (buf ^ 1) * CHUNK_BYTES + wave * kPanelPieceBytes;
+        bool scratch_used = false;
         while (need_drain || nredo > 0 || (k + 1 == ntot && qcount > 0)) {
-            drain();
+#if MCE_PANEL_STATS
+            const long long t_w0 = clock64();
+#endif
+            if (!scratch_used) asm volatile("s_waitcnt vmcnt(0)" ::: "memory");
+#if MCE_PANEL_STATS
+            st_tW += clock64() - t_w0;
+            st_ends += scratch_used ? 0 : 1;
+#endif
+            scratch_used = true;
+            drain(scr);
             need_drain = false;
             const int n = nredo;
             nredo = 0;
@@ -624,6 +620,17 @@
 #endif
             }
         }
+        if (scratch_used && k + 1 < ntot) {
+#if MCE_PANEL_STATS
+            const long long t_s0 = clock64();
+#endif
+            asm volatile("s_waitcnt lgkmcnt(0)" ::: "memory");
+            stage_async(c + 1, buf ^ 1);
+#if MCE_PANEL_STATS
+            asm volatile("s_waitcnt vmcnt(0)" ::: "memory");
+            st_tS += clock64() - t_s0;
+#endif
+        }
     }
 
 #if MCE_PANEL_STATS
@@ -633,7 +640,7 @@
         o[0] = (double)st_drains; o[1] = (double)st_enq; o[2] = (double)st_redo; o[3] = (double)st_events;
         o[4] = (double)st_tE; o[5] = (double)st_tD; o[6] = (double)(clock64() - t_kernel0); o[7] = (double)st_tPro;
         double* o2 = const_cast<double*>(a->params) + 16 + ((int64_t)gridDim.x * kHWaves) * 8 + ((int64_t)blockIdx.x * kHWaves + wave) * 8;
-        o2[0] = (double)st_tA; o2[1] = (double)st_tR; o2[2] = (double)(st_tD - st_tA - st_tR); o2[3] = (double)st_tB; o2[4] = 0; o2[5] = 0; o2[6] = 0; o2[7] = 0;
+        o2[0] = (double)st_tA; o2[1] = (double)st_tR; o2[2] = (double)(st_tD - st_tA - st_tR); o2[3] = (double)st_tB; o2[4] = (double)st_tW; o2[5] = (double)st_tS; o2[6] = (double)st_ends; o2[7] = 0;
     }
 #endif
     {
diff --git a/mcevidence_amd/csrc/panel_geom.hpp b/mcevidence_amd/csrc/panel_geom.hpp
--- /dev/null
+++ b/mcevidence_amd/csrc/panel_geom.hpp
@@ -0,0 +1,58 @@
+#pragma once
+#include <stddef.h>
+
+#include "sym_types.hpp"
+
+#ifndef MCE_PANEL_STAGE_KB
+#define MCE_PANEL_STAGE_KB 64
+#endif
+#ifndef MCE_PANEL_QUEUE
+#define MCE_PANEL_QUEUE 640
+#endif
+#ifndef MCE_PANEL_TRIGGER
+#define MCE_PANEL_TRIGGER 384
+#endif
+
+namespace mce {
+
+constexpr int kPanelWaves = 8;
+constexpr int kPanelPieceBytes = 64 * 16;
+constexpr int kPanelPieceStride = kPanelWaves * kPanelPieceBytes;
+constexpr int kPanelScratchEntryBytes = 12;
+
+MCE_HD constexpr int panel_chunk_tiles(int KST)
+{
+    int ct = MCE_PANEL_STAGE_KB / KST < 64 ? MCE_PANEL_STAGE_KB / KST : 64;
+    ct = ct / 2 * 2;
+    while (ct > 2 && (ct * KST) % 8 != 0) ct -= 2;
+    return ct;
+}
+MCE_HD constexpr int panel_wave_pieces(int KST) { return panel_chunk_tiles(KST) * KST / kPanelWaves; }
+MCE_HD constexpr int panel_queue(int KST)
+{
+    const int cap = panel_wave_pieces(KST) * kPanelPieceBytes / kPanelScratchEntryBytes / 64 * 64;
+    if (KST == 3) return 448 < cap ? 448 : cap;
+    return MCE_PANEL_QUEUE < cap ? MCE_PANEL_QUEUE : cap;
+}
+MCE_HD constexpr int panel_trigger(int KST)
+{
+    if (KST == 3) return 192;
+    return MCE_PANEL_TRIGGER < panel_queue(KST) - 128 ? MCE_PANEL_TRIGGER : panel_queue(KST) - 128;
+}
+
+MCE_HD constexpr int panel_scratch_offset(int wave, int entry, int field, int qn)
+{
+    const unsigned lin = field == 0 ? 8u * (unsigned)entry : 8u * (unsigned)qn + 4u * (unsigned)entry;
+    return wave * kPanelPieceBytes + (int)(lin / kPanelPieceBytes) * kPanelPieceStride + (int)(lin % kPanelPieceBytes);
+}
+
+MCE_HD constexpr size_t panel_lds_bytes(int KST)
+{
+    return (size_t)2 * panel_chunk_tiles(KST) * KST * 1024
+           + (size_t)kPanelWaves * panel_queue(KST) * 4
+           + (size_t)kPanelWaves * 2 * 32 * 4 + 128
+           + (size_t)kPanelWaves * 2 * 32 * 4
+           + (size_t)kPanelWaves * panel_chunk_tiles(KST) * 2 * 4;
+}
+
+}
```

New measurement: 26.61 million (median of 4 runs). About the same (+0.3%).
